# lijx10/SO-Net

Measured on AMD Instinct MI355X. Metric: point-clouds/sec forward, ModelNet40 5k-pt 8x8 SOM, higher is better.
Workload: dtype f32 (operands split into fp16 pieces, 3 fp16 MFMAs per product, f32 accumulate; parity 1e-5)

## Files before the change

include/sonet_hip.h:

```cpp
#ifndef SONET_HIP_H
#define SONET_HIP_H

#include <stddef.h>
#include <stdint.h>

#ifdef __cplusplus
extern "C" {
#endif

typedef void *sonet_stream_t;

enum {
    SONET_OK = 0,
    SONET_ERR_INVALID_ARG = 1,
    SONET_ERR_UNSUPPORTED = 2,
    SONET_ERR_LAUNCH = 3,
    SONET_ERR_NO_DEVICE = 4
};

int sonet_abi_version(void);
const char *sonet_build_arch(void);
const char *sonet_last_error(void);
int sonet_check_device(void);
int sonet_diag_mfma_f16_rate(int random_operands, int iters, double *tflops_out, double *ghz_out, sonet_stream_t stream);

int sonet_range_log_set(uint32_t *slot);

int sonet_index_max_f32(const float *data, const int32_t *index, int32_t *out_idx,
                        int B, int C, int Np, int K, sonet_stream_t stream);
int sonet_index_max_bf16(const uint16_t *data, const int32_t *index, int32_t *out_idx,
                         int B, int C, int Np, int K, sonet_stream_t stream);
int sonet_index_max_gather_f32(const float *data, const int32_t *index, const int32_t *row_max,
                               int32_t *out_idx, float *out_val,
                               int B, int C, int Np, int K, sonet_stream_t stream);
int sonet_index_max_gather_bf16(const uint16_t *data, const int32_t *index, const int32_t *row_max,
                                int32_t *out_idx, float *out_val, int B, int C, int Np, int K,
                                sonet_stream_t stream);
int sonet_index_max_gather_p16(const void *planes, const int32_t *index, const int32_t *row_max,
                               int32_t *out_idx, float *out_val, int B, int C, int Np, int K, sonet_stream_t stream);

int sonet_som_assign_f32(const float *x, const float *node, int B, int N, int M, int k,
                         int32_t *min_idx_i32, int64_t *min_idx_i64, int32_t *count, double *sum_ws,
                         sonet_stream_t stream);

int sonet_som_group_f32(const float *x, const float *sn, const int32_t *min_idx_i32,
                        const int32_t *count, const double *sum_ws, int B, int N, int M, int k,
                        float *som_node, int32_t *row_max, float *centers, float *x_decentered,
                        float *x_augmented, sonet_stream_t stream);

#define SONET_SOM_TRAIN_MAX_NODES 1024
#define SONET_SOM_TRAIN_MAX_POINTS (1 << 28)
int sonet_som_train_f32(const float *x, const float *node0, int node0_shared, const float *w, const float *lr,
                        int T, int B, int N, int M, float *node_out, sonet_stream_t stream);

int sonet_som_mask_i32(const int32_t *min_idx_i32, int32_t *mask, int B, int kN, int M,
                       sonet_stream_t stream);

int sonet_node_gather_f32(const float *feat, const int32_t *min_idx_i32, float *out,
                          int B, int C, int M, int kN, sonet_stream_t stream);

int sonet_knn_gather_f32(const float *x, const int64_t *knn_I, float *out,
                         int B, int C, int M, int K, sonet_stream_t stream);

int sonet_knn_self_f32(const float *node, int64_t *knn_I, int B, int M, int K, sonet_stream_t stream);

#define SONET_BATCH_SHAPENET 1
#define SONET_BATCH_TRAIN 2
#define SONET_BATCH_ROT_HORIZONTAL 4
#define SONET_BATCH_ROT_PERTURBATION 8
#define SONET_BATCH_TRANSLATION 16
#define SONET_BATCH_FLAG_MASK 31
#define SONET_BATCH_DRAW_SCALARS 8
#define SONET_BATCH_MAX_K 16
int sonet_assemble_batch_f32(const float *src, long long P, const int64_t *offsets, int S, const float *nodes_src,
                             const int64_t *idx, int B, int N, int M, int K, int flags, long long seed,
                             long long step, const int64_t *replay_idx, const double *replay_draws, double *draws_out,
                             float *pc, float *sn, float *node, int64_t *chosen, int64_t *knn_I, int32_t *bad,
                             sonet_stream_t stream);

int sonet_knn_group_f32(const float *coord, const float *feat, const int64_t *knn_I, int B, int C, int M, int K,
                        int center_avg, float *center, float *out, sonet_stream_t stream);
int sonet_knn_prepare_f32(const float *coord, const int64_t *knn_I, int B, int M, int K, int center_avg,
                          float *center, float *dec, int32_t *gidx, sonet_stream_t stream);
int sonet_pointmlp_h3_gather_f32(const float *x1, int C1, int L1, const int32_t *gidx, const float *x2, int C2, const void *Wp3,
                                 const float *scale, const float *shift, int relu, float *y,
                                 int B, int Cout, int L, sonet_stream_t stream);
int sonet_planes_max_f32(const float *x, float *out, long long rows, int K, int M, sonet_stream_t stream);

int sonet_lastdim_max_f32(const float *x, float *out, long long rows, int K, sonet_stream_t stream);

size_t sonet_pointmlp_pack_size(int Cin, int Cout);
int sonet_pointmlp_pack_f32(const float *W, float *Wp, int Cin, int Cout, sonet_stream_t stream);
int sonet_pointmlp_f32(const float *x1, int C1, const float *x2, int C2, const float *Wp,
                       const float *scale, const float *shift, int relu, float *y,
                       int B, int Cout, int L, sonet_stream_t stream);

int sonet_pointmlp_x3_bnb_f32(const float *gy, const float *raw, int C, const void *Wp3, const float *scale, const float *shift,
                              const float *a, const float *b, const float *c0, const float *sc, const float *sh, int relu,
                              float *g_raw_out, float *y, int B, int Cout, int L,
                              const float *praw, const float *psc, const float *psh, int prelu, void *pstats_ws, double *psums,
                              sonet_stream_t stream);

int sonet_pointmlp_x3_bnb_acc_f32(const float *gy, const float *raw, int C, const void *Wp3, const float *scale, const float *shift,
                                  const float *a, const float *b, const float *c0, const float *sc, const float *sh, int relu,
                                  float *g_raw_out, const float *yadd, float *y, int B, int Cout, int L, sonet_stream_t stream);

size_t sonet_pointmlp_x3_pack_size(int Cin, int Cout);
int sonet_pointmlp_x3_pack(const float *W, void *Wp3, int Cin, int Cout, sonet_stream_t stream);
int sonet_pointmlp_x3_f32(const float *x1, int C1, const float *x2, int C2, const void *Wp3,
                          const float *scale, const float *shift, int relu, float *y,
                          int B, int Cout, int L, sonet_stream_t stream);

int sonet_pointmlp_h3_pack(const float *W, void *Wp3, int Cin, int Cout, sonet_stream_t stream);
int sonet_pointmlp_h3_f32(const float *x1, int C1, const float *x2, int C2, const void *Wp3,
                          const float *scale, const float *shift, int relu, float *y,
                          int B, int Cout, int L, sonet_stream_t stream);

size_t sonet_p16_size(int B, int C, int L);
int sonet_p16_from_f32(const float *x, void *p16, int B, int C, int L, const float *scale, const float *shift, int relu,
                       sonet_stream_t stream);
int sonet_p16_to_f32(const void *p16, float *x, int B, int C, int L, sonet_stream_t stream);
size_t sonet_pointmlp_h3p_pack_size(int Cin, int Cout);
int sonet_pointmlp_h3p_pack(const float *W, void *Wp, int Cin, int Cout, sonet_stream_t stream);
size_t sonet_pointmlp_h3p_stats_ws_size(int B, int Cout, int L);
int sonet_pointmlp_h3p(const void *x1p, int C1, int L1, const int32_t *gidx, const void *x2p, int C2, const void *Wp,
                       const float *scale, const float *shift, int relu, float *y, void *yp, int B, int Cout, int L,
                       const float *zadd, const int32_t *zidx, int ZM, void *stats_ws, float *mean, float *var,
                       sonet_stream_t stream);

size_t sonet_knn_stage_columns(int B, int M, int K);
size_t sonet_node_stage_columns(int B, int M);
int sonet_knn_stage_prepare_f32(const float *coord, const int64_t *knn_I, int KI, int center_avg, int B, int M, int K,
                                float *center, void *center_p16, void *rec, sonet_stream_t stream);
int sonet_knn_stage_input_p16(const void *rec, const void *z_p16, const float *wl, const float *scale, const float *shift, int relu,
                              int B, int M, int K, int C, void *h1_p16, sonet_stream_t stream);
int sonet_pointmlp_h3p_gmax(const void *x1p, int C1, const void *x2p, int C2, const void *Wp, const float *scale, const float *shift,
                            int relu, int Cout, int L, int GK, int G, int ngout, int Lout, float *y, void *yp, sonet_stream_t stream);
int sonet_p16_flat_to_bcm_f32(const void *p16, float *x, int B, int C, int M, sonet_stream_t stream);

int sonet_lastdim_argmax_f32(const float *x, float *out, int32_t *idx, long long rows, int K, sonet_stream_t stream);
int sonet_lastdim_argmax_bf16(const uint16_t *x, uint16_t *out, int32_t *idx, long long rows, int K, sonet_stream_t stream);
int sonet_lastdim_max_bwd_f32(const float *g, const int32_t *idx, float *gx, long long rows, int K, sonet_stream_t stream);
int sonet_lastdim_max_bwd_bf16(const uint16_t *g, const int32_t *idx, uint16_t *gx, long long rows, int K, sonet_stream_t stream);
size_t sonet_knn_gather_bwd_ws_size(int B, int M, int K);
int sonet_knn_gather_bwd_f32(const float *g, const int64_t *knn_I, float *gx, void *ws, int B, int C, int M, int K, sonet_stream_t stream);
int sonet_knn_gather_bwd_bf16(const uint16_t *g, const int64_t *knn_I, float *gx, void *ws, int B, int C, int M, int K, sonet_stream_t stream);
size_t sonet_node_gather_bwd_ws_size(int B, int M, int L);
int sonet_node_gather_bwd_f32(const float *g, const int32_t *ids, float *gx, void *ws, int B, int C, int M, int L, sonet_stream_t stream);
int sonet_node_gather_bwd_bf16(const uint16_t *g, const int32_t *ids, float *gx, void *ws, int B, int C, int M, int L, sonet_stream_t stream);
size_t sonet_pointwise_bwd_apply_nodesum_ws_size(int B, int M, int L);
int sonet_pointwise_bwd_apply_nodesum_tile(void);
int sonet_pointwise_bwd_apply_nodesum_f32(const float *gy, const float *raw, const float *scale, const float *shift, int relu,
                                          const float *a, const float *b, const float *c0, const int32_t *ids, int M,
                                          float *g_raw, float *gz, void *ws, int B, int C, int L, sonet_stream_t stream);

size_t sonet_pointmlp_bf16_pack_size(int Cin, int Cout);
int sonet_pointmlp_bf16_pack(const float *W, void *Wp, int Cin, int Cout, sonet_stream_t stream);
int sonet_pointmlp_bf16(const uint16_t *x1, int C1, const uint16_t *x2, int C2, const void *Wp,
                        const float *scale, const float *shift, int relu, uint16_t *y,
                        int B, int Cout, int L, sonet_stream_t stream);
int sonet_pointmlp_bf16_gather(const uint16_t *x1, int C1, int L1, const int32_t *gidx, const uint16_t *x2, int C2, const void *Wp,
                               const float *scale, const float *shift, int relu, uint16_t *y,
                               int B, int Cout, int L, sonet_stream_t stream);
int sonet_pointmlp_bf16_acc(const uint16_t *x1, int C1, const uint16_t *x2, int C2, const void *Wp,
                            const float *scale, const float *shift, int relu, const uint16_t *yadd, uint16_t *y,
                            int B, int Cout, int L, sonet_stream_t stream);
int sonet_pointmlp_bf16_bnb(const uint16_t *gy, const uint16_t *raw, int C, const void *Wp, const float *scale, const float *shift,
                            const float *a, const float *b, const float *c0, const float *sc, const float *sh, int relu,
                            uint16_t *g_raw_out, const uint16_t *yadd, uint16_t *y, int B, int Cout, int L, sonet_stream_t stream);

size_t sonet_pointresnet_pack_size(void);
int sonet_pointresnet_pack(const float *W1, const float *W2, const float *W3, const float *W4, int Cin0,
                           void *wstream, sonet_stream_t stream);
int sonet_pointresnet_fused_f32(const float *x, int Cin0, const void *wstream, const float *affine,
                                float *y, int B, int L, sonet_stream_t stream);
int sonet_pointresnet_fused_p16_f32(const float *x, int Cin0, const void *wstream, const float *affine,
                                    float *y, void *yp, int B, int L, sonet_stream_t stream);

size_t sonet_pointresnet_bf16_pack_size(void);
int sonet_pointresnet_bf16_pack(const float *W1, const float *W2, const float *W3, const float *W4, int Cin0,
                                void *wstream, sonet_stream_t stream);
int sonet_pointresnet_bf16(const float *x, int Cin0, const void *wstream, const float *affine,
                           uint16_t *y, int B, int L, sonet_stream_t stream);

size_t sonet_pointresnet_bf16_pool_ws_size(int B, int L, int M);
int sonet_pointresnet_bf16_pool(const float *x_sorted, int Cin0, const void *wstream, const float *affine,
                                const int32_t *ids_sorted, const int32_t *pos0, const int32_t *node_off,
                                const int32_t *count, void *ws, float *out, int B, int L, int M, sonet_stream_t stream);

size_t sonet_pointresnet_pool_ws_size(int B, int L, int M);
int sonet_pointresnet_fused_pool_f32(const float *x_sorted, int Cin0, const void *wstream, const float *affine,
                                     const int32_t *ids_sorted, const int32_t *pos0, const int32_t *node_off,
                                     const int32_t *count, void *ws, float *out, int B, int L, int M, sonet_stream_t stream);
int sonet_pointresnet_fused_pool_p16_f32(const float *x_sorted, int Cin0, const void *wstream, const float *affine,
                                         const int32_t *ids_sorted, const int32_t *pos0, const int32_t *node_off,
                                         const int32_t *count, void *ws, float *out, void *out_p16, int B, int L, int M, sonet_stream_t stream);
size_t sonet_som_assign_sort_ws_size(int B, int N, int M, int k);
int sonet_som_assign_sort_f32(const float *x, const float *sn, const float *node, int B, int N, int M, int k,
                              int32_t *min_idx_i32, int64_t *min_idx_i64, int32_t *count, double *sum_ws,
                              float *som_node, int32_t *row_max, float *x_aug_sorted, int32_t *ids_sorted,
                              int32_t *pos0, int32_t *node_off, void *ws, sonet_stream_t stream);
int sonet_som_assign_sort_det_f32(const float *x, const float *sn, const float *node, int B, int N, int M, int k,
                              int32_t *min_idx_i32, int64_t *min_idx_i64, int32_t *count, double *sum_ws,
                              float *som_node, int32_t *row_max, float *x_aug_sorted, int32_t *ids_sorted,
                              int32_t *pos0, int32_t *node_off, void *ws, sonet_stream_t stream);
int sonet_som_assign_sort_knn_f32(const float *x, const float *sn, const float *node, int B, int N, int M, int k,
                                  int32_t *min_idx_i32, int64_t *min_idx_i64, int32_t *count, double *sum_ws,
                                  float *som_node, int32_t *row_max, float *x_aug_sorted, int32_t *ids_sorted,
                                  int32_t *pos0, int32_t *node_off, void *ws,
                                  const int64_t *knn_I, int KI, int K, int center_avg, float *center, void *center_p16, void *rec,
                                  sonet_stream_t stream);
int sonet_som_sort_group_f32(const float *x, const float *sn, const int32_t *min_idx_i32, const int32_t *count,
                             const double *sum_ws, int B, int N, int M, int k, float *som_node, int32_t *row_max,
                             float *x_aug_sorted, int32_t *ids_sorted, int32_t *pos0, int32_t *node_off,
                             int32_t *cursor_ws, sonet_stream_t stream);

int sonet_channel_stats_bf16(const uint16_t *y, int B, int C, int L, double *stat_ws, float *mean, float *var, sonet_stream_t stream);
int sonet_channel_affine_act_out_bf16(const uint16_t *x, const float *scale, const float *shift, int relu, uint16_t *y,
                                      int B, int C, int L, sonet_stream_t stream);
int sonet_pointwise_bwd_stats_bf16(const uint16_t *gy, const uint16_t *raw, const float *scale, const float *shift,
                                   int relu, int B, int C, int L, double *sums, sonet_stream_t stream);
int sonet_pointwise_bwd_apply_bf16(const uint16_t *gy, const uint16_t *raw, const float *scale, const float *shift, int relu,
                                   const float *a, const float *b, const float *c0, uint16_t *g_raw, int B, int C, int L,
                                   sonet_stream_t stream);

int sonet_pointwise_bwd_stats_f32(const float *gy, const float *raw, const float *scale, const float *shift,
                                  int relu, int B, int C, int L, double *sums, sonet_stream_t stream);
int sonet_pointwise_bwd_apply_f32(const float *gy, const float *raw, const float *scale, const float *shift, int relu,
                                  const float *a, const float *b, const float *c0, float *g_raw,
                                  int B, int C, int L, sonet_stream_t stream);
int sonet_node_add_affine_act_f32(float *t, const float *z, const int32_t *min_idx_i32, const float *scale,
                                  const float *shift, int relu, int B, int C, int L, int M, sonet_stream_t stream);

size_t sonet_pointmlp_stats_ws_size(int B, int Cout, int L);
int sonet_pointmlp_h3_stats_f32(const float *x1, int C1, const float *x2, int C2, const void *Wp3, const float *scale,
                                const float *shift, int relu, float *y, int B, int Cout, int L, void *stats_ws,
                                float *mean, float *var, sonet_stream_t stream);
int sonet_pointmlp_x3_stats_f32(const float *x1, int C1, const float *x2, int C2, const void *Wp3, const float *scale,
                                const float *shift, int relu, float *y, int B, int Cout, int L, void *stats_ws,
                                float *mean, float *var, sonet_stream_t stream);

int sonet_pointmlp_h3_nodeadd_f32(const float *x1, int C1, const float *x2, int C2, const void *Wp3, const float *scale,
                                  const float *shift, int relu, float *y, int B, int Cout, int L,
                                  const float *zadd, const int32_t *zidx, int ZM, sonet_stream_t stream);
int sonet_pointmlp_h3_nodeadd_stats_f32(const float *x1, int C1, const float *x2, int C2, const void *Wp3, const float *scale,
                                        const float *shift, int relu, float *y, int B, int Cout, int L,
                                        const float *zadd, const int32_t *zidx, int ZM, void *stats_ws,
                                        float *mean, float *var, sonet_stream_t stream);

size_t sonet_pointmlp_bf16_stats_ws_size(int B, int Cout, int L);
int sonet_pointmlp_bf16_stats(const uint16_t *x1, int C1, const uint16_t *x2, int C2, const void *Wp,
                              const float *scale, const float *shift, int relu, uint16_t *y,
                              int B, int Cout, int L, void *stats_ws, float *mean, float *var, sonet_stream_t stream);
int sonet_pointmlp_bf16_pool(const uint16_t *x1, int C1, const uint16_t *x2, int C2, const void *Wp,
                             const float *scale, const float *shift, int relu, const int32_t *ids, const int32_t *row_max,
                             int32_t *out_idx, float *out_val, int B, int Cout, int L, int M, sonet_stream_t stream);
int sonet_pointmlp_bf16_stats_xaff(const uint16_t *x1, int C1, const uint16_t *x2, int C2, const void *Wp,
                                   const float *scale, const float *shift, int relu, uint16_t *y,
                                   int B, int Cout, int L, void *stats_ws, float *mean, float *var,
                                   const float *xs1, const float *xh1, const float *xs2, const float *xh2, int xrelu,
                                   sonet_stream_t stream);
int sonet_pointmlp_bf16_pool_xaff(const uint16_t *x1, int C1, const uint16_t *x2, int C2, const void *Wp,
                                  const float *scale, const float *shift, int relu, const int32_t *ids, const int32_t *row_max,
                                  int32_t *out_idx, float *out_val, int B, int Cout, int L, int M,
                                  const float *xs1, const float *xh1, const float *xs2, const float *xh2, int xrelu,
                                  sonet_stream_t stream);

size_t sonet_pointmlp_h3_segpool_ws_size(int B, int Cout, int M);
int sonet_pointmlp_h3_segpool_f32(const float *x1, int C1, const float *x2, int C2, const void *Wp3, const float *scale,
                                  const float *shift, int relu, const int32_t *ids_sorted, const int32_t *pos0,
                                  const int32_t *row_max, int M, void *ws, int32_t *out_idx, float *out_val,
                                  int B, int Cout, int L, const float *xs1, const float *xh1, const float *xs2, const float *xh2,
                                  int xrelu, sonet_stream_t stream);
int sonet_pointmlp_h3_stats_xaff_f32(const float *x1, int C1, const float *x2, int C2, const void *Wp3, const float *scale,
                                     const float *shift, int relu, float *y, int B, int Cout, int L, void *stats_ws,
                                     float *mean, float *var, const float *xs1, const float *xh1, const float *xs2, const float *xh2,
                                     int xrelu, sonet_stream_t stream);

size_t sonet_wgrad_x3_ws_size(int B, int Cout, int Cin, int L);
int sonet_wgrad_x3_f32(const float *g, const float *x, float *dw, void *ws, int B, int Cout, int Cin, int L, sonet_stream_t stream);
int sonet_wgrad_x3_xaff_f32(const float *g, const float *x, float *dw, void *ws, int B, int Cout, int Cin, int L,
                            const float *xs, const float *xh, int xrelu, sonet_stream_t stream);
size_t sonet_wgrad_bf16_ws_size(int B, int Cout, int Cin, int L);
int sonet_wgrad_bf16(const uint16_t *g, const uint16_t *x, float *dw, void *ws, int B, int Cout, int Cin, int L, sonet_stream_t stream);
int sonet_wgrad_bf16_xaff(const uint16_t *g, const uint16_t *x, float *dw, void *ws, int B, int Cout, int Cin, int L,
                          const float *xs, const float *xh, int xrelu, sonet_stream_t stream);
int sonet_node_gather_lead_affine_act_f32(const float *z, const int32_t *gidx, const float *lead, const float *wl,
                                          const float *scale, const float *shift, int relu, float *out,
                                          int B, int C, int L, int M, int NL, sonet_stream_t stream);

// ... 122 lines not shown
```

so-net_amd/csrc/device.hpp:

```cpp
#pragma once
#include <hip/hip_runtime.h>
#include <stdint.h>
#include <type_traits>

typedef float f32x2_t __attribute__((ext_vector_type(2)));
typedef float f32x4_t __attribute__((ext_vector_type(4)));
typedef float f32x16 __attribute__((ext_vector_type(16)));
typedef _Float16 f16x2_t __attribute__((ext_vector_type(2)));
typedef _Float16 f16x8 __attribute__((ext_vector_type(8)));
typedef __bf16 bf16x8 __attribute__((ext_vector_type(8)));
typedef short i16x2 __attribute__((ext_vector_type(2)));
typedef int i32x4_t __attribute__((ext_vector_type(4)));
typedef unsigned u32x4_t __attribute__((ext_vector_type(4)));

template <int V> using int_c = std::integral_constant<int, V>;
template <bool B> using bool_c = std::integral_constant<bool, B>;

__device__ __forceinline__ unsigned cvt_pk_bf16(float lo, float hi) {
    unsigned r;
    asm("v_cvt_pk_bf16_f32 %0, %1, %2" : "=v"(r) : "v"(lo), "v"(hi));
    return r;
}
__device__ __forceinline__ unsigned cvt_pk_f16(float lo, float hi) {
    const f32x2_t v = {lo, hi};
    return __builtin_bit_cast(unsigned, __builtin_convertvector(v, f16x2_t));
}
__device__ __forceinline__ unsigned ord_f32(unsigned bits) {
    if (bits == 0x80000000u) bits = 0u;
    const unsigned o = bits ^ ((unsigned)((int)bits >> 31) | 0x80000000u);
    return (bits & 0x7FFFFFFFu) > 0x7F800000u ? 0u : o;
}

constexpr int RAW_BUFFER_WORD3 = 0x00020000;
template <typename T>
__device__ __forceinline__ __amdgpu_buffer_rsrc_t raw_buffer(const T *ptr, int bytes) {
    return __builtin_amdgcn_make_buffer_rsrc(const_cast<T *>(ptr), 0, bytes, RAW_BUFFER_WORD3);
}
__device__ __forceinline__ i32x4_t raw_buffer_sgpr(const void *base, unsigned bytes) {
    const unsigned long long a = reinterpret_cast<unsigned long long>(base);
    i32x4_t r;
    r[0] = __builtin_amdgcn_readfirstlane((int)(unsigned)a);
    r[1] = __builtin_amdgcn_readfirstlane((int)(unsigned)((a >> 32) & 0xFFFFu));
    r[2] = __builtin_amdgcn_readfirstlane((int)bytes);
    r[3] = RAW_BUFFER_WORD3;
    return r;
}

__device__ __forceinline__ float ld_f32(const float *p, long long i) { return p[i]; }
__device__ __forceinline__ float ld_f32(const uint16_t *p, long long i) { return __uint_as_float((unsigned)p[i] << 16); }
__device__ __forceinline__ void st_rne(float *p, long long i, float v) { p[i] = v; }
__device__ __forceinline__ void st_rne(uint16_t *p, long long i, float v) { p[i] = (uint16_t)(cvt_pk_bf16(v, v) & 0xFFFFu); }
__device__ __forceinline__ void st4_rne(float *o, const float (&v)[4]) { *reinterpret_cast<float4 *>(o) = make_float4(v[0], v[1], v[2], v[3]); }
__device__ __forceinline__ void st4_rne(uint16_t *o, const float (&v)[4]) {
    *reinterpret_cast<uint2 *>(o) = make_uint2(cvt_pk_bf16(v[0], v[1]), cvt_pk_bf16(v[2], v[3]));
}

__device__ __forceinline__ unsigned bf16_pair_affine_act(unsigned pk, f32x2_t sc, f32x2_t sh, unsigned floor2) {
    const f32x2_t x = {__uint_as_float(pk << 16), __uint_as_float(pk & 0xFFFF0000u)};
    f32x2_t v;
    asm("v_pk_fma_f32 %0, %1, %2, %3" : "=v"(v) : "v"(x), "v"(sc), "v"(sh));
    unsigned r = cvt_pk_bf16(v[0], v[1]);
    asm("v_pk_max_i16 %0, %1, %2" : "=v"(r) : "v"(r), "v"(floor2));
    return r;
}

__device__ __forceinline__ float row32_sum(float v) {
    v += __builtin_bit_cast(float, __builtin_amdgcn_update_dpp(0, __builtin_bit_cast(int, v), 0xB1, 0xF, 0xF, true));
    v += __builtin_bit_cast(float, __builtin_amdgcn_update_dpp(0, __builtin_bit_cast(int, v), 0x4E, 0xF, 0xF, true));
    v += __builtin_bit_cast(float, __builtin_amdgcn_update_dpp(0, __builtin_bit_cast(int, v), 0x141, 0xF, 0xF, true));
    v += __builtin_bit_cast(float, __builtin_amdgcn_update_dpp(0, __builtin_bit_cast(int, v), 0x140, 0xF, 0xF, true));
    v += __builtin_bit_cast(float, __builtin_amdgcn_ds_swizzle(__builtin_bit_cast(int, v), 0x401F));
    return v;
}

__device__ __forceinline__ int xcd_remap(int bid, int nwg) {
    const int q = nwg / sonet::NUM_XCD, r = nwg % sonet::NUM_XCD;
    const int xcd = bid % sonet::NUM_XCD, local = bid / sonet::NUM_XCD;
    const int base = xcd < r ? xcd * (q + 1) : r * (q + 1) + (xcd - r) * q;
    return base + local;
}

struct RangeAcc { int mp; unsigned mn; };
__device__ __forceinline__ void range_track(RangeAcc &r, float x0, float x1) {
    const int a = __float_as_int(x0), b = __float_as_int(x1);
    r.mp = max(max(r.mp, a), b);
    r.mn = max(max(r.mn, (unsigned)a), (unsigned)b);
}
__device__ __forceinline__ unsigned range_amax_bits(const RangeAcc &r) {
    const unsigned neg = (r.mn & 0x80000000u) ? (r.mn & 0x7FFFFFFFu) : 0u;
    const unsigned pos = (unsigned)r.mp;
    return pos > neg ? pos : neg;
}
__device__ __forceinline__ unsigned wave_umax(unsigned v) {
#pragma unroll
    for (int o = 32; o > 0; o >>= 1) { const unsigned t = (unsigned)__shfl_xor((int)v, o, 64); v = t > v ? t : v; }
    return v;
}
__device__ __forceinline__ void range_publish(unsigned *word, unsigned wave_max_bits, int lane) {
    if (lane == 0 && wave_max_bits > __atomic_load_n(word, __ATOMIC_RELAXED)) atomicMax(word, wave_max_bits);
}

__device__ __forceinline__ void p16_split2(float X0, float X1, unsigned &h, unsigned &m) {
    h = cvt_pk_f16(X0, X1);
    const f16x2_t hv = __builtin_bit_cast(f16x2_t, h);
    m = cvt_pk_f16(X0 - (float)hv[0], X1 - (float)hv[1]);
}
__device__ __forceinline__ void p16_split_pair(float x0, float x1, unsigned &h, unsigned &m) {
    p16_split2(32.f * __builtin_amdgcn_fmed3f(x0, -2047.f, 2047.f), 32.f * __builtin_amdgcn_fmed3f(x1, -2047.f, 2047.f), h, m);
}
__device__ __forceinline__ float clamp_keep_nan(float w, float lim) { return w < -lim ? -lim : (w > lim ? lim : w); }
__device__ __forceinline__ int p16_channel(int h, int e) { return 4 * h + (e & 3) + 8 * (e >> 2); }

__device__ __forceinline__ void split3_pair(float x0, float x1, unsigned &h, unsigned &m, unsigned &l) {
    h = cvt_pk_bf16(x0, x1);
    const float r0 = x0 - __uint_as_float(h << 16), r1 = x1 - __uint_as_float(h & 0xFFFF0000u);
    m = cvt_pk_bf16(r0, r1);
    const float q0 = r0 - __uint_as_float(m << 16), q1 = r1 - __uint_as_float(m & 0xFFFF0000u);
    l = cvt_pk_bf16(q0, q1);
}

__device__ __forceinline__ void split3_fix_w(float w, unsigned &h, unsigned &m, unsigned &l) {
    if ((h & 0x7FFFu) != 0x7F80u) return;
    if (__builtin_isinf(w)) { l = h; h = 0u; m = 0u; return; }
    h -= 1u;
    const float r = w - __uint_as_float(h << 16);
    m = cvt_pk_bf16(r, 0.f) & 0xFFFFu;
    l = cvt_pk_bf16(r - __uint_as_float(m << 16), 0.f) & 0xFFFFu;
}
__device__ __forceinline__ void split3_pair_w(float w0, float w1, unsigned &h, unsigned &m, unsigned &l) {
    split3_pair(w0, w1, h, m, l);
    unsigned h0 = h & 0xFFFFu, m0 = m & 0xFFFFu, l0 = l & 0xFFFFu, h1 = h >> 16, m1 = m >> 16, l1 = l >> 16;
    split3_fix_w(w0, h0, m0, l0);
    split3_fix_w(w1, h1, m1, l1);
    h = h0 | (h1 << 16); m = m0 | (m1 << 16); l = l0 | (l1 << 16);
}

__device__ __forceinline__ float cluster_mean(float sum, float count) { return __fdiv_rn(sum, __fadd_rn(count, 1e-5f)); }
```

so-net_amd/csrc/node_stage.hip:

```cpp
#include "common.hpp"

namespace {

constexpr int KS_CPW = 4;

__global__ __launch_bounds__(256) void knn_stage_prepare_kernel(const float *__restrict__ coord, const int64_t *__restrict__ I, int KI, int avg,
                                                                 int B, int M, int K, int G, long long Lp, long long Lm,
                                                                 float *__restrict__ center, uint4 *__restrict__ center_p16, int4 *__restrict__ rec,
                                                                 unsigned *__restrict__ rlog)
{
    const long long l = (long long)blockIdx.x * 256 + threadIdx.x;
    if (l >= Lp) return;
    const int col = (int)(l & 127);
    const long long BM = (long long)B * M;
    const int g = col / K, k = col - g * K;
    const long long n = (l >> 7) * G + g;
    if (!(g < G && n < BM)) {
        rec[l] = make_int4(-2, 0, 0, 0);
        return;
    }
    const int b = (int)(n / M), m = (int)(n - (long long)b * M);
    const int64_t *Ib = I + ((long long)b * M + m) * KI;
    const float *cb = coord + (long long)b * 3 * M;
    const long long id = Ib[k];
    const bool ok = (unsigned long long)id < (unsigned long long)M;
    float d[3], ctr[3];
#pragma unroll
    for (int c = 0; c < 3; ++c) {
        const float *src = cb + c * M;
        if (avg) {
            float sum = 0.f;
            for (int kk = 0; kk < K; ++kk) {
                const long long ik = Ib[kk];
                sum += ((unsigned long long)ik < (unsigned long long)M) ? src[ik] : 0.f;
            }
            ctr[c] = sum / (float)K;
        } else {
            ctr[c] = src[m];
        }
        d[c] = (ok ? src[id] : 0.f) - ctr[c];
    }
    rec[l] = make_int4(ok ? (int)((long long)b * M + id) : -1, __float_as_int(d[0]), __float_as_int(d[1]), __float_as_int(d[2]));
    if (k == 0) {
#pragma unroll
        for (int c = 0; c < 3; ++c) center[((long long)b * 3 + c) * M + m] = ctr[c];
        unsigned h0, m0, h1v, m1;
        p16_split_pair(ctr[0], ctr[1], h0, m0);
        p16_split_pair(ctr[2], 0.f, h1v, m1);
        center_p16[(0 * 2 + 0) * Lm + n] = make_uint4(h0, h1v, 0u, 0u);
        center_p16[(0 * 2 + 1) * Lm + n] = make_uint4(0u, 0u, 0u, 0u);
        center_p16[(1 * 2 + 0) * Lm + n] = make_uint4(m0, m1, 0u, 0u);
        center_p16[(1 * 2 + 1) * Lm + n] = make_uint4(0u, 0u, 0u, 0u);
        if (rlog != nullptr) {
            RangeAcc xr = {0, 0u};
            range_track(xr, ctr[0], ctr[1]);
            range_track(xr, ctr[2], 0.f);
            const unsigned bits = range_amax_bits(xr);
            if (bits > __atomic_load_n(rlog + 2, __ATOMIC_RELAXED)) atomicMax(rlog + 2, bits);
        }
    }
}


constexpr int KS_MAXG = 8;

__global__ __launch_bounds__(256) void knn_stage_input_kernel(const int4 *__restrict__ rec, const uint4 *__restrict__ zp, const float *__restrict__ wl,
                                                               const float *__restrict__ scale, const float *__restrict__ shift, int relu,
                                                               int C, long long Lp, long long Lm, uint4 *__restrict__ h1, unsigned *__restrict__ rlog, int abl)
{
    __shared__ unsigned wmax[4];
    __shared__ __attribute__((aligned(16))) float coef[5][KS_MAXG * KS_CPW * 16];
    const int col = threadIdx.x & 127;
    const int hh = __builtin_amdgcn_readfirstlane((int)(threadIdx.x >> 7));
    const long long lcol = (long long)blockIdx.x * 128 + col;
    const int4 r = rec[lcol];
    const int KC = (C + 15) >> 4;
    const int ngrp = (KC + KS_CPW - 1) / KS_CPW, gstride = (int)gridDim.y;
    for (int t = threadIdx.x; t < KS_MAXG * KS_CPW * 16; t += 256) {
        const int j = t >> 6, i = (t >> 4) & 3, h = (t >> 3) & 1, e = t & 7;
        const int grp = (int)blockIdx.y + j * gstride;
        const int c = (grp * KS_CPW + i) * 16 + p16_channel(h, e);
        const bool in = grp < ngrp && c < C;
        coef[0][t] = in ? 32.f * wl[c * 3 + 0] : 0.f;
        coef[1][t] = in ? 32.f * wl[c * 3 + 1] : 0.f;
        coef[2][t] = in ? 32.f * wl[c * 3 + 2] : 0.f;
        coef[3][t] = in ? scale[c] : 0.f;
        coef[4][t] = in ? 32.f * shift[c] : 0.f;
    }
    const bool valid = r.x != -2, ok = r.x >= 0;
    const f32x2_t d0 = {__int_as_float(r.y), __int_as_float(r.y)}, d1 = {__int_as_float(r.z), __int_as_float(r.z)},
                d2 = {__int_as_float(r.w), __int_as_float(r.w)};
    RangeAcc xr = {0, 0u};
    const float lo = relu ? 0.f : -65504.f;
    const uint4 *zbase = zp + (long long)hh * Lm + (ok ? r.x : 0);
    uint4 *hbase = h1 + (long long)hh * Lp + lcol;

    auto load = [&](uint4 (&zh)[KS_CPW], uint4 (&zm)[KS_CPW], int grp) {
        const uint4 *zq = zbase + (long long)(grp * KS_CPW) * 4 * Lm;
#pragma unroll
        for (int i = 0; i < KS_CPW; ++i) {
            zh[i] = make_uint4(0u, 0u, 0u, 0u);
            zm[i] = zh[i];
#ifdef SONET_VARIANTS
            if (abl & 2) { zh[i] = make_uint4(r.y, r.z, r.w, r.x); zm[i] = zh[i]; } else
#endif
            if (ok && grp * KS_CPW + i < KC) {
                zh[i] = zq[0];
                zm[i] = zq[2 * Lm];
            }
            zq += 4 * Lm;
        }
    };
    auto process = [&](const uint4 (&zhq)[KS_CPW], const uint4 (&zmq)[KS_CPW], int grp, int j) {
        uint4 *hq = hbase + (long long)(grp * KS_CPW) * 4 * Lp;
#pragma unroll
        for (int i = 0; i < KS_CPW; ++i) {
            if (grp * KS_CPW + i >= KC) break;
            const unsigned zh[4] = {zhq[i].x, zhq[i].y, zhq[i].z, zhq[i].w}, zm[4] = {zmq[i].x, zmq[i].y, zmq[i].z, zmq[i].w};
            unsigned hv[4], mv[4];
#pragma unroll
            for (int q = 0; q < 4; ++q) {
                const int slot = (j * KS_CPW + i) * 16 + hh * 8 + 2 * q;
                const f32x2_t w0 = *reinterpret_cast<const f32x2_t *>(&coef[0][slot]), w1 = *reinterpret_cast<const f32x2_t *>(&coef[1][slot]),
                            w2 = *reinterpret_cast<const f32x2_t *>(&coef[2][slot]), sc = *reinterpret_cast<const f32x2_t *>(&coef[3][slot]),
                            sh = *reinterpret_cast<const f32x2_t *>(&coef[4][slot]);
                const f16x2_t zh2 = __builtin_bit_cast(f16x2_t, zh[q]), zm2 = __builtin_bit_cast(f16x2_t, zm[q]);
                f32x2_t a = __builtin_convertvector(zh2, f32x2_t) + __builtin_convertvector(zm2, f32x2_t);
                a = __builtin_elementwise_fma(w0, d0, a);
                a = __builtin_elementwise_fma(w1, d1, a);
                a = __builtin_elementwise_fma(w2, d2, a);
                a = __builtin_elementwise_fma(a, sc, sh);
                if (!valid) a = f32x2_t{0.f, 0.f};
                range_track(xr, a[0], a[1]);
                p16_split2(__builtin_amdgcn_fmed3f(a[0], lo, 65504.f), __builtin_amdgcn_fmed3f(a[1], lo, 65504.f), hv[q], mv[q]);
            }
#ifdef SONET_VARIANTS
            if ((abl & 1) && hv[0] != 0x12345u) { hq += 4 * Lp; continue; }
#endif
            hq[0] = make_uint4(hv[0], hv[1], hv[2], hv[3]);
            hq[2 * Lp] = make_uint4(mv[0], mv[1], mv[2], mv[3]);
            hq += 4 * Lp;
        }
    };

    uint4 zhA[KS_CPW], zmA[KS_CPW], zhB[KS_CPW], zmB[KS_CPW];
    int grp = (int)blockIdx.y, j = 0;
    load(zhA, zmA, grp);
    __syncthreads();
    for (; grp < ngrp; grp += 2 * gstride, j += 2) {
        const bool more = grp + gstride < ngrp;
        if (more) load(zhB, zmB, grp + gstride);
        process(zhA, zmA, grp, j);
        if (more) {
            if (grp + 2 * gstride < ngrp) load(zhA, zmA, grp + 2 * gstride);
            process(zhB, zmB, grp + gstride, j + 1);
        }
    }
    if (rlog != nullptr) {
        unsigned bits;
        if (relu) {
            const unsigned pos = xr.mp > 0 ? (unsigned)xr.mp : 0u, nan_neg = xr.mn > 0xFF800000u ? (xr.mn & 0x7FFFFFFFu) : 0u;
            bits = pos > nan_neg ? pos : nan_neg;
        } else {
            bits = range_amax_bits(xr);
        }
        unsigned wm = wave_umax(bits);
        wm = wm > (5u << 23) ? wm - (5u << 23) : 0u;
        if ((threadIdx.x & 63) == 0) wmax[threadIdx.x >> 6] = wm;
        __syncthreads();
        if (threadIdx.x == 0) {
            const unsigned a = wmax[0] > wmax[1] ? wmax[0] : wmax[1], c2 = wmax[2] > wmax[3] ? wmax[2] : wmax[3];
            const unsigned mx = a > c2 ? a : c2;
            if (mx > __atomic_load_n(rlog + 2, __ATOMIC_RELAXED)) atomicMax(rlog + 2, mx);
        }
    }
}

__global__ __launch_bounds__(256) void p16_flat_to_bcm_kernel(const uint4 *__restrict__ p, float *__restrict__ x, int C, int M, long long BM, long long Lm, int KC)
{
    const long long l = (long long)blockIdx.x * 256 + threadIdx.x;
    const int kc = blockIdx.y >> 1, hh = blockIdx.y & 1;
    if (l >= BM) return;
    const uint4 hv = p[((long long)(kc * 2 + 0) * 2 + hh) * Lm + l], mv = p[((long long)(kc * 2 + 1) * 2 + hh) * Lm + l];
    const f16x8 h8 = __builtin_bit_cast(f16x8, hv), m8 = __builtin_bit_cast(f16x8, mv);
    const long long b = l / M;
    const int m = (int)(l - b * M);
#pragma unroll
    for (int e = 0; e < 8; ++e) {
        const int c = kc * 16 + p16_channel(hh, e);
        if (c < C) x[(b * C + c) * M + m] = ((float)h8[e] + (float)m8[e]) * 0.03125f;
    }
}

}

extern "C" size_t sonet_knn_stage_columns(int B, int M, int K)
{
    if (B <= 0 || M <= 0 || K <= 0 || K > 128) return 0;
    return (size_t)(sonet::ceil_div64((long long)B * M, knn_stage_groups(K)) * 128);
}

extern "C" size_t sonet_node_stage_columns(int B, int M)
{
    if (B <= 0 || M <= 0) return 0;
    return (size_t)(sonet::ceil_div64((long long)B * M, 128) * 128);
}

extern "C" int sonet_knn_stage_prepare_f32(const float *coord, const int64_t *knn_I, int KI, int center_avg, int B, int M, int K,
                                           float *center, void *center_p16, void *rec, sonet_stream_t stream)
{
    const char *what = "sonet_knn_stage_prepare_f32";
    SONET_REQUIRE(coord && knn_I && center && center_p16 && rec, "%s: NULL pointer", what);
    SONET_REQUIRE(B > 0 && M > 0 && K >= 1 && K <= 128 && KI >= K, "%s: bad size B=%d M=%d K=%d (of %d)", what, B, M, K, KI);
    const long long Lp = (long long)sonet_knn_stage_columns(B, M, K), Lm = (long long)sonet_node_stage_columns(B, M);
    if (Lp / 256 + 1 > 0x7FFFFFFFll) return sonet::fail(SONET_ERR_UNSUPPORTED, "%s: too many columns", what);
    hipLaunchKernelGGL(knn_stage_prepare_kernel, dim3((unsigned)sonet::ceil_div64(Lp, 256)), dim3(256), 0, sonet::as_stream(stream),
                       coord, knn_I, KI, center_avg, B, M, K, knn_stage_groups(K), Lp, Lm, center, reinterpret_cast<uint4 *>(center_p16),
                       reinterpret_cast<int4 *>(rec), sonet::range_log());
    return sonet::launched(what);
}

extern "C" int sonet_knn_stage_input_p16(const void *rec, const void *z_p16, const float *wl, const float *scale, const float *shift, int relu,
                                         int B, int M, int K, int C, void *h1_p16, sonet_stream_t stream)
{
    const char *what = "sonet_knn_stage_input_p16";
    SONET_REQUIRE(rec && z_p16 && wl && scale && shift && h1_p16, "%s: NULL pointer", what);
    SONET_REQUIRE(B > 0 && M > 0 && C > 0 && K >= 1 && K <= 128, "%s: bad size B=%d M=%d C=%d K=%d", what, B, M, C, K);
    const long long Lp = (long long)sonet_knn_stage_columns(B, M, K), Lm = (long long)sonet_node_stage_columns(B, M);
    const long long nblk = Lp / 128;
    const int KC = sonet::ceil_div(C, 16);
    if (nblk > 0x7FFFFFFFll || (double)KC * 64.0 * (double)Lp >= 2.0e9) return sonet::fail(SONET_ERR_UNSUPPORTED, "%s: too many columns", what);
    const int ngrp = sonet::ceil_div(KC, KS_CPW);
    int gy = sonet::ceil_div(ngrp, KS_MAXG);
    while (gy < ngrp && nblk * gy < 512) ++gy;
#ifdef SONET_VARIANTS
    if (const char *e = sonet::knob("SONET_KSI_GY")) { const int v = atoi(e); if (v >= sonet::ceil_div(ngrp, KS_MAXG) && v <= ngrp) gy = v; }
#endif
    hipLaunchKernelGGL(knn_stage_input_kernel, dim3((unsigned)nblk, (unsigned)gy), dim3(256), 0, sonet::as_stream(stream),
                       reinterpret_cast<const int4 *>(rec), reinterpret_cast<const uint4 *>(z_p16), wl, scale, shift, relu, C, Lp, Lm,
                       reinterpret_cast<uint4 *>(h1_p16), sonet::range_log(), sonet::knob("SONET_KSI_ABL") ? atoi(sonet::knob("SONET_KSI_ABL")) : 0);
    return sonet::launched(what);
}

extern "C" int sonet_p16_flat_to_bcm_f32(const void *p16, float *x, int B, int C, int M, sonet_stream_t stream)
{
    const char *what = "sonet_p16_flat_to_bcm_f32";
    SONET_REQUIRE(p16 && x, "%s: NULL pointer", what);
    SONET_REQUIRE(B > 0 && C > 0 && M > 0, "%s: non-positive size", what);
    const int KC = sonet::ceil_div(C, 16);
    const long long BM = (long long)B * M;
    if (KC * 2 > 65535) return sonet::fail(SONET_ERR_UNSUPPORTED, "%s: C too large for one launch", what);
    hipLaunchKernelGGL(p16_flat_to_bcm_kernel, dim3((unsigned)sonet::ceil_div64(BM, 256), (unsigned)(KC * 2)), dim3(256), 0, sonet::as_stream(stream),
                       reinterpret_cast<const uint4 *>(p16), x, C, M, BM, (long long)sonet_node_stage_columns(B, M), KC);
    return sonet::launched(what);
}
```

so-net_amd/csrc/pointmlp_h3p.hip:

```cpp
#include "common.hpp"

namespace {

constexpr int P_THREADS = 256;
constexpr int P_KPAD = 8;
constexpr unsigned OOB = 0x7FFFFF00u;

template <bool RELU>
__device__ __forceinline__ void split_act(float x0, float x1, unsigned &h, unsigned &m) {
    constexpr float lo = RELU ? 0.f : -2047.f;
    p16_split2(32.f * __builtin_amdgcn_fmed3f(x0, lo, 2047.f), 32.f * __builtin_amdgcn_fmed3f(x1, lo, 2047.f), h, m);
}

__global__ __launch_bounds__(256) void h3p_pack_kernel(const float *__restrict__ W, uint4 *__restrict__ Wp, int Cin, int Cout, int KCP,
                                                        long long total, unsigned *__restrict__ trailer)
{
    const long long t = (long long)blockIdx.x * 256 + threadIdx.x;
    if (t >= total) return;
    RangeAcc wr = {0, 0u};
    const int lane = (int)(t & 63);
    const long long r = t >> 6;
    const int kc = (int)(r % KCP), ct = (int)(r / KCP);
    const int o = ct * 32 + (lane & 31), hh = lane >> 5;
    unsigned h[4], m[4];
#pragma unroll
    for (int p = 0; p < 4; ++p) {
        const int c0 = kc * 16 + p16_channel(hh, 2 * p), c1 = c0 + 1;
        float w0 = (o < Cout && c0 < Cin) ? W[(long long)o * Cin + c0] : 0.f;
        float w1 = (o < Cout && c1 < Cin) ? W[(long long)o * Cin + c1] : 0.f;
        range_track(wr, w0, w1);
        w0 = 32.f * clamp_keep_nan(w0, 2047.f);
        w1 = 32.f * clamp_keep_nan(w1, 2047.f);
        p16_split2(w0, w1, h[p], m[p]);
    }
    uint4 *dst = Wp + (r * 2) * 64 + lane;
    dst[0] = make_uint4(h[0], h[1], h[2], h[3]);
    dst[64] = make_uint4(m[0], m[1], m[2], m[3]);
    range_publish(trailer, wave_umax(range_amax_bits(wr)), lane);
}

template <bool AFFINE>
__global__ __launch_bounds__(256) void p16_from_f32_kernel(const float *__restrict__ x, uint4 *__restrict__ p, int C, int L, int KC,
                                                            const float *__restrict__ scale, const float *__restrict__ shift, int relu,
                                                            unsigned *__restrict__ rlog)
{
    __shared__ unsigned wmax[4];
    const int kc = blockIdx.y >> 1, hh = blockIdx.y & 1, b = blockIdx.z;
    RangeAcc xr = {0, 0u};
    const float *xb0 = x + (size_t)b * C * L;
    uint4 *pb = p + (size_t)b * KC * 4 * L;
    float sc[8], sf[8];
    if constexpr (AFFINE) {
#pragma unroll
        for (int e = 0; e < 8; ++e) {
            const int c = kc * 16 + p16_channel(hh, e);
            sc[e] = c < C ? scale[c] : 0.f;
            sf[e] = c < C ? shift[c] : 0.f;
        }
    }
#pragma unroll
    for (int it = 0; it < 4; ++it) {
        const int l = blockIdx.x * 1024 + it * 256 + threadIdx.x;
        if (l >= L) break;
        const float *xb = xb0 + l;
        float v[8];
#pragma unroll
        for (int e = 0; e < 8; ++e) {
            const int c = kc * 16 + p16_channel(hh, e);
            float t = c < C ? xb[(size_t)c * L] : 0.f;
            if constexpr (AFFINE) {
                t = __fmaf_rn(t, sc[e], sf[e]);
                if (relu) t = t < 0.f ? 0.f : t;
            }
            v[e] = t;
        }
        unsigned h[4], m[4];
#pragma unroll
        for (int q = 0; q < 4; ++q) {
            range_track(xr, v[2 * q], v[2 * q + 1]);
            split_act<false>(v[2 * q], v[2 * q + 1], h[q], m[q]);
        }
        pb[((size_t)(kc * 2 + 0) * 2 + hh) * L + l] = make_uint4(h[0], h[1], h[2], h[3]);
        pb[((size_t)(kc * 2 + 1) * 2 + hh) * L + l] = make_uint4(m[0], m[1], m[2], m[3]);
    }
    if (rlog != nullptr) {
        const unsigned wm = wave_umax(range_amax_bits(xr));
        if ((threadIdx.x & 63) == 0) wmax[threadIdx.x >> 6] = wm;
        __syncthreads();
        if (threadIdx.x == 0) {
            const unsigned a = wmax[0] > wmax[1] ? wmax[0] : wmax[1], c2 = wmax[2] > wmax[3] ? wmax[2] : wmax[3];
            const unsigned mx = a > c2 ? a : c2;
            if (mx > __atomic_load_n(rlog + 2, __ATOMIC_RELAXED)) atomicMax(rlog + 2, mx);
        }
    }
}

__global__ __launch_bounds__(256) void p16_to_f32_kernel(const uint4 *__restrict__ p, float *__restrict__ x, int C, int L, int KC)
{
    const int l = blockIdx.x * 256 + threadIdx.x;
    const int kc = blockIdx.y >> 1, hh = blockIdx.y & 1, b = blockIdx.z;
    if (l >= L) return;
    const uint4 *pb = p + (size_t)b * KC * 4 * L;
    const uint4 hv = pb[((size_t)(kc * 2 + 0) * 2 + hh) * L + l], mv = pb[((size_t)(kc * 2 + 1) * 2 + hh) * L + l];
    const f16x8 h8 = __builtin_bit_cast(f16x8, hv), m8 = __builtin_bit_cast(f16x8, mv);
    float *xb = x + (size_t)b * C * L + l;
#pragma unroll
    for (int e = 0; e < 8; ++e) {
        const int c = kc * 16 + p16_channel(hh, e);
        if (c < C) xb[(size_t)c * L] = ((float)h8[e] + (float)m8[e]) * 0.03125f;
    }
}

struct H3pArgs {
    const void *x1, *x2;
    const void *Wp;
    const float *scale, *shift;
    float *y;
    void *yp;
    const int32_t *gidx;
    const float *zadd;
    const int32_t *zidx;
    unsigned *rlog;
    double *stats_partial;
    int abl;
    unsigned long long *prof;
    long long ngroups;
    int KC1, KC2, L1, L, Cout, CT, KC, KCr, KCP, ct_per_y, nslab, ncol, gpc, relu, ZM;
    int GK, G, ngout, Lout;
};

__device__ __forceinline__ u32x4_t bload16(i32x4_t rsrc, unsigned voff, unsigned soff) {
    u32x4_t r;
    asm volatile("buffer_load_dwordx4 %0, %1, %2, %3 offen" : "=v"(r) : "v"(voff), "s"(rsrc), "s"(soff) : "memory");
    return r;
}
__device__ __forceinline__ void bstore16(__amdgpu_buffer_rsrc_t rsrc, unsigned voff, unsigned soff, u32x4_t v) {
    __builtin_amdgcn_raw_buffer_store_b128(v, rsrc, voff, soff, 0);
}
__device__ __forceinline__ void bstore4(__amdgpu_buffer_rsrc_t rsrc, unsigned voff, unsigned soff, float v) {
    __builtin_amdgcn_raw_buffer_store_b32(__builtin_bit_cast(unsigned, v), rsrc, voff, soff, 0);
}
template <int N>
__device__ __forceinline__ void wait_barrier(u32x4_t &a, u32x4_t &b) {
    asm volatile("s_waitcnt vmcnt(%2)\n\ts_barrier" : "+v"(a), "+v"(b) : "n"(N) : "memory");
}
template <int N>
__device__ __forceinline__ void wait_barrier(u32x4_t &a, u32x4_t &b, u32x4_t &c, u32x4_t &d) {
    asm volatile("s_waitcnt vmcnt(%4)\n\ts_barrier" : "+v"(a), "+v"(b), "+v"(c), "+v"(d) : "n"(N) : "memory");
}

template <int NC>
__device__ __forceinline__ void sched_pair() {
    __builtin_amdgcn_sched_group_barrier(0x100, 1, 0);
    __builtin_amdgcn_sched_group_barrier(0x008, NC == 2 ? 3 : 1, 0);
    __builtin_amdgcn_sched_group_barrier(0x100, 1, 0);
    __builtin_amdgcn_sched_group_barrier(0x008, NC == 2 ? 3 : 2, 0);
    __builtin_amdgcn_sched_group_barrier(0x100, 1, 0);
    __builtin_amdgcn_sched_group_barrier(0x008, NC == 2 ? 3 : 1, 0);
    __builtin_amdgcn_sched_group_barrier(0x100, 1, 0);
    __builtin_amdgcn_sched_group_barrier(0x008, NC == 2 ? 3 : 2, 0);
}

constexpr int GM_STRIDE = 136;
__device__ __forceinline__ float nan_max(float m, float v) { return (v > m || v != v) ? v : m; }
__device__ __forceinline__ void lds_barrier() { asm volatile("s_waitcnt lgkmcnt(0)\n\ts_barrier" ::: "memory"); }

template <int MT, int NC, int OCC, int EPI, int OUT>
__global__ __launch_bounds__(P_THREADS, OCC) void pointmlp_h3p_kernel(const H3pArgs a)
{
    static_assert(OUT >= 1 && OUT <= 3 && (EPI != 2 || (OUT & 1)), "output mode");
    static_assert(EPI < 4 || (NC == 1 && ((EPI == 4 && OUT == 2) || (EPI == 5 && OUT == 1))), "group-max epilogues: 32-column waves, P16 (4) or f32 (5) out");
    static_assert(MT % 2 == 0 && (NC == 1 || NC == 2), "tile shape");
    constexpr int PB = (OCC >= 2 && NC == 2 && (EPI == 1 || EPI == 3)) ? 2 : 3, NB = 4, D = 3, NSLOT = D + 2;
    static_assert(D >= PB && PB >= 2, "the wait count below assumes the W request of a chunk is older than its X request");
    constexpr int NSL = MT * 2;
    constexpr int ND = NSL / 4;
    constexpr int NBL = NC * 2;
    constexpr int NP = MT / 2;
    constexpr int KWAIT = (PB - 1) * (NBL + ND);
    static_assert(KWAIT < 64, "vmcnt is a 6-bit counter");
    struct Lds {
        u32x4_t wsm[NSLOT][NSL][64];
        float aff[EPI == 1 ? 1024 : 2048];
        float2 red[EPI == 2 ? 4 : 1][EPI == 2 ? MT * 32 : 1];
        float zl[EPI == 1 ? MT * 32 : 1][EPI == 1 ? 64 : 1];
        float gm[EPI >= 4 ? 32 : 1][EPI >= 4 ? GM_STRIDE : 1];
    };
    __shared__ __attribute__((aligned(16))) Lds lds;

    const int wg_xcd = blockIdx.x & 7, wg_local = blockIdx.x >> 3;
    const int wg_col = (wg_local / a.nslab) * 8 + wg_xcd, wg_slab = wg_local - (wg_local / a.nslab) * a.nslab;
    if (wg_col >= a.ncol) return;

    const int lane = threadIdx.x & 63;
    const int wave = __builtin_amdgcn_readfirstlane(threadIdx.x >> 6);
    const int j = lane & 31, h = lane >> 5;
    long long q = (long long)wg_col * 4 + wave;
    const bool wave_valid = q < a.ngroups;
    q = wave_valid ? q : 0;
    const int b = __builtin_amdgcn_readfirstlane((int)(q / a.gpc));
    const int l0 = __builtin_amdgcn_readfirstlane((int)(q - (long long)b * a.gpc) * (32 * NC));
    const int L = a.L, L1 = a.L1;

    bool pv[NC];
    unsigned vo1[NC], vo2[NC], voy[NC], voyp[NC];
    int lcl[NC];
#pragma unroll
    for (int c = 0; c < NC; ++c) {
        const int l = l0 + 32 * c + j;
        pv[c] = wave_valid && l < L;
        lcl[c] = l < L ? l : l0;
        vo2[c] = (unsigned)(h * L + lcl[c]) * 16u;
        vo1[c] = (unsigned)(h * L1 + lcl[c]) * 16u;
        if (a.gidx) {
            const int src = a.gidx[(size_t)b * L + lcl[c]];
            vo1[c] = (unsigned)src < (unsigned)L1 ? (unsigned)(h * L1 + src) * 16u : OOB;
        }
        voy[c] = pv[c] ? (unsigned)(4 * h * L + l) * 4u : OOB;
        voyp[c] = pv[c] ? (unsigned)(h * L + l) * 16u : OOB;
#ifdef SONET_VARIANTS
        if (a.abl & 1) { voy[c] = OOB; voyp[c] = OOB; pv[c] = false; }
#endif
    }
    const i32x4_t r1 = raw_buffer_sgpr(static_cast<const char *>(a.x1) + (size_t)b * a.KC1 * 64 * L1, (unsigned)a.KC1 * 64u * (unsigned)L1);
    const i32x4_t r2 = raw_buffer_sgpr(a.x2 ? static_cast<const char *>(a.x2) + (size_t)b * a.KC2 * 64 * L : static_cast<const char *>(a.x1),
                                 a.x2 ? (unsigned)a.KC2 * 64u * (unsigned)L : 0u);
    const __amdgpu_buffer_rsrc_t ry = __builtin_amdgcn_make_buffer_rsrc(
        a.y ? reinterpret_cast<char *>(a.y) + (size_t)b * a.Cout * L * 4 : nullptr, 0, a.y ? (int)((unsigned)a.Cout * (unsigned)L * 4u) : 0, RAW_BUFFER_WORD3);
    const __amdgpu_buffer_rsrc_t ryp = __builtin_amdgcn_make_buffer_rsrc(
        a.yp ? static_cast<char *>(a.yp) + (size_t)b * (a.Cout / 16) * 64 * L : nullptr, 0, a.yp ? (int)((unsigned)(a.Cout / 16) * 64u * (unsigned)L) : 0, RAW_BUFFER_WORD3);

    const int ct_begin = wg_slab * a.ct_per_y;
    const int ct_end = min(a.CT, ct_begin + a.ct_per_y);
    const int npass = (ct_end - ct_begin) / MT;
    const int KCr = a.KCr, KC1 = a.KC1;
#ifdef SONET_VARIANTS
    unsigned long long pt0 = __builtin_readcyclecounter(), pt_loop = 0, pt_epi = 0, pt_pro = 0;
#endif
    const unsigned wsm_lds = (unsigned)reinterpret_cast<size_t>(&lds.wsm[0][0][0]);
    const unsigned vow = (unsigned)lane * 16u;
    const char *wp = static_cast<const char *>(a.Wp);

    auto load_b = [&](u32x4_t (&bb)[NBL], int kc) {
#ifdef SONET_VARIANTS
        if (a.abl & 2) kc = 0;
#endif
        const bool second = kc >= KC1;
        const int kk = second ? kc - KC1 : kc;
        const unsigned rowb = (unsigned)(second ? L : L1) * 32u;
        const i32x4_t rs = second ? r2 : r1;
#pragma unroll
        for (int c = 0; c < NC; ++c) {
            const unsigned vo = second ? vo2[c] : vo1[c];
            bb[2 * c + 0] = bload16(rs, vo, (unsigned)(kk * 2 + 0) * rowb);
            bb[2 * c + 1] = bload16(rs, vo, (unsigned)(kk * 2 + 1) * rowb);
        }
    };
    auto dma = [&](int pass, int kc, int slot) {
#ifdef SONET_VARIANTS
        if (a.abl & 4) { kc = 0; pass = 0; }
#endif
        const int ps = pass < npass ? pass : npass - 1;
        const char *g0 = wp + ((size_t)(ct_begin + ps * MT) * a.KCP + kc) * 2048u;
        const unsigned d0 = wsm_lds + (unsigned)slot * (unsigned)(NSL * 1024);
#pragma unroll
        for (int t = 0; t < ND; ++t) {
            const int sl = wave + 4 * t;
            const char *g = g0 + (size_t)(sl >> 1) * ((size_t)a.KCP * 2048u) + (size_t)(sl & 1) * 1024u;
            const unsigned d = d0 + (unsigned)sl * 1024u;
            unsigned keep;
            asm volatile("s_mov_b32 %0, m0\n\ts_mov_b32 m0, %3\n\ts_nop 4\n\tglobal_load_lds_dwordx4 %1, %2\n\ts_mov_b32 m0, %0"
                         : "=&s"(keep) : "v"(vow), "s"(g), "s"(d) : "memory");
        }
    };
    auto read_a = [&](u32x4_t (&A)[4], int slot, int p) {
#pragma unroll
        for (int u = 0; u < 4; ++u) A[u] = lds.wsm[slot][4 * p + u][lane];
    };

    f32x16 acc[MT][NC];

    auto mfma_pair = [&](const u32x4_t (&A)[4], const u32x4_t (&bb)[NBL], int p) {
        f16x8 Bh[NC], Bm[NC];
#pragma unroll
        for (int c = 0; c < NC; ++c) {
            Bh[c] = __builtin_bit_cast(f16x8, bb[2 * c + 0]);
            Bm[c] = __builtin_bit_cast(f16x8, bb[2 * c + 1]);
        }
#pragma unroll
        for (int term = 0; term < 3; ++term)
#pragma unroll
            for (int tt = 0; tt < 2; ++tt)
#pragma unroll
                for (int c = 0; c < NC; ++c)
                {
                    const f16x8 wf = __builtin_bit_cast(f16x8, A[2 * tt + (term == 0 ? 1 : 0)]), xf = term == 1 ? Bm[c] : Bh[c];
                    acc[2 * p + tt][c] = __builtin_amdgcn_mfma_f32_32x32x16_f16(wf, xf, acc[2 * p + tt][c], 0, 0, 0);
                }
    };

    RangeAcc yr = {0, 0u};
    const float relu_thr = a.relu ? 0.f : -__builtin_inff();
    const float split_lo = a.relu ? 0.f : -2047.f;
    int zm[NC];
    bool zok[NC];
    unsigned zvo[NC], zla[NC];
    const i32x4_t rz = raw_buffer_sgpr(a.zadd ? a.zadd + (size_t)b * a.Cout * a.ZM : nullptr, a.zadd ? (unsigned)a.Cout * (unsigned)a.ZM * 4u : 0u);
    if constexpr (EPI == 1 || EPI == 3) {
#pragma unroll
        for (int c = 0; c < NC; ++c) {
            zm[c] = a.zidx[(size_t)b * L + lcl[c]];
            zok[c] = (unsigned)zm[c] < (unsigned)a.ZM;
            zm[c] = zok[c] ? zm[c] : 0;
            zvo[c] = zok[c] ? (unsigned)(zm[c] + 4 * h * a.ZM) * 4u : OOB;
            zla[c] = (unsigned)reinterpret_cast<size_t>(&lds.zl[4 * h][zm[c]]);
            asm volatile("" : "+v"(zla[c]));
        }
    }
    auto epilogue = [&](int ct0) {
        if constexpr (EPI >= 4) {
#pragma unroll
            for (int mt = 0; mt < MT; ++mt) {
                if ((ct0 + mt) * 32 >= a.Cout) continue;
                float asc16[16], ash16[16];
                {
                    const float4 *t4 = reinterpret_cast<const float4 *>(lds.aff + (ct0 - ct_begin + mt) * 64 + h * 32);
#pragma unroll
                    for (int u = 0; u < 4; ++u) {
                        const float4 s4 = t4[u], h4 = t4[4 + u];
                        asc16[4 * u] = s4.x; asc16[4 * u + 1] = s4.y; asc16[4 * u + 2] = s4.z; asc16[4 * u + 3] = s4.w;
                        ash16[4 * u] = h4.x; ash16[4 * u + 1] = h4.y; ash16[4 * u + 2] = h4.z; ash16[4 * u + 3] = h4.w;
                    }
                }
                __builtin_amdgcn_sched_barrier(0);
#pragma unroll
                for (int r = 0; r < 16; ++r) {
                    const float v = __fmaf_rn(acc[mt][0][r], asc16[r], ash16[r]);
                    lds.gm[(r & 3) + 8 * (r >> 2) + 4 * h][32 * wave + j] = v < relu_thr ? 0.f : v;
                }
                lds_barrier();
                const int t = (int)threadIdx.x;
                if constexpr (EPI == 4) {
                    const int p = t & 3, u = t >> 2;
                    const int g = u % a.G, qh = u / a.G;
                    if (qh < 4) {
                        const int qq = qh >> 1, h2 = qh & 1;
                        const float *r0 = &lds.gm[16 * qq + 4 * h2 + 2 * (p & 1) + 8 * (p >> 1)][g * a.GK];
                        float m0 = r0[0], m1 = r0[GM_STRIDE];
                        for (int k = 1; k < a.GK; ++k) {
                            m0 = nan_max(m0, r0[k]);
                            m1 = nan_max(m1, r0[GM_STRIDE + k]);
                        }
                        const long long n_out = (long long)wg_col * a.G + g;
                        if (n_out < a.ngout) {
                            range_track(yr, m0, m1);
                            unsigned hv, mv;
                            p16_split2(__builtin_amdgcn_fmed3f(m0, split_lo * 32.f, 65504.f), __builtin_amdgcn_fmed3f(m1, split_lo * 32.f, 65504.f), hv, mv);
                            unsigned *dst = reinterpret_cast<unsigned *>(static_cast<char *>(a.yp)
                                + ((((size_t)((ct0 + mt) * 2 + qq) * 2) * 2 + h2) * (size_t)a.Lout + (size_t)n_out) * 16) + p;
                            dst[0] = hv;
                            dst[(size_t)a.Lout * 8] = mv;
                        }
                    }
                } else {
                    const int seg = t & 3, row = (t >> 2) & 31, g = t >> 7;
                    const int cols = a.GK >> 2;
                    const float *r0 = &lds.gm[row][(g < a.G ? g : 0) * a.GK + seg * cols];
                    float m = r0[0];
                    for (int k = 1; k < cols; ++k) m = nan_max(m, r0[k]);
                    m = nan_max(m, __builtin_bit_cast(float, __builtin_amdgcn_update_dpp(0, __builtin_bit_cast(int, m), 0xB1, 0xF, 0xF, true)));
                    m = nan_max(m, __builtin_bit_cast(float, __builtin_amdgcn_update_dpp(0, __builtin_bit_cast(int, m), 0x4E, 0xF, 0xF, true)));
                    const long long n_out = (long long)wg_col * a.G + g;
                    if (seg == 0 && g < a.G && n_out < a.ngout) a.y[(size_t)n_out * a.Cout + (size_t)(ct0 + mt) * 32 + row] = m;
                }
                lds_barrier();
            }
            return;
        }
#pragma unroll
        for (int mt = 0; mt < MT; ++mt) {
            if ((ct0 + mt) * 32 >= a.Cout) continue;
            float asc16[16], ash16[16];
            {
                const float4 *t4 = reinterpret_cast<const float4 *>(lds.aff + (ct0 - ct_begin + mt) * 64 + h * 32);
#pragma unroll
                for (int u = 0; u < 4; ++u) {
                    const float4 s4 = t4[u], h4 = t4[4 + u];
                    asc16[4 * u] = s4.x; asc16[4 * u + 1] = s4.y; asc16[4 * u + 2] = s4.z; asc16[4 * u + 3] = s4.w;
                    ash16[4 * u] = h4.x; ash16[4 * u + 1] = h4.y; ash16[4 * u + 2] = h4.z; ash16[4 * u + 3] = h4.w;
                }
            }
            __builtin_amdgcn_sched_barrier(0);
            float st1[EPI == 2 ? 16 : 1], st2[EPI == 2 ? 16 : 1];
#pragma unroll
            for (int c = 0; c < NC; ++c) {
#pragma unroll
                for (int qq = 0; qq < 2; ++qq) {
                    unsigned hh[4], mm[4];
#pragma unroll
                    for (int hf = 0; hf < 2; ++hf) {
                        const int r0 = 8 * qq + 4 * hf;
                        const int row0 = mt * 32 + 16 * qq + 8 * hf;
                        float av[4], v[4], zg[4];
#pragma unroll
                        for (int e = 0; e < 4; ++e) {
                            if constexpr (OCC == 1) asm volatile("v_accvgpr_read_b32 %0, %1" : "=v"(av[e]) : "a"(acc[mt][c][r0 + e]));
                            else av[e] = acc[mt][c][r0 + e];
                        }
                        if constexpr (EPI == 3) {
#pragma unroll
                            for (int e = 0; e < 4; ++e) {
                                const unsigned so = (unsigned)((ct0 + mt) * 32 + 16 * qq + 8 * hf + e) * (unsigned)a.ZM * 4u;
                                asm volatile("buffer_load_dword %0, %1, %2, %3 offen" : "=v"(zg[e]) : "v"(zvo[c]), "s"(rz), "s"(so) : "memory");
                            }
                            asm volatile("s_waitcnt vmcnt(0)" : "+v"(zg[0]), "+v"(zg[1]), "+v"(zg[2]), "+v"(zg[3]) :: "memory");
                        }
                        if constexpr (EPI == 1) {
#pragma unroll
                            for (int e = 0; e < 4; ++e)
                                asm volatile("v_add_u32 %0, %2, %1\n\tds_read_b32 %0, %0" : "=&v"(zg[e]) : "v"(zla[c]), "s"((row0 + e) * 256) : "memory");
                            asm volatile("s_waitcnt lgkmcnt(0)" : "+v"(zg[0]), "+v"(zg[1]), "+v"(zg[2]), "+v"(zg[3]) :: "memory");
                        }
#pragma unroll
                        for (int e = 0; e < 4; ++e) {
                            const float sc = asc16[r0 + e], sf = ash16[r0 + e];
                            if constexpr (EPI == 1 || EPI == 3) {
                                const float zv = EPI == 1 ? (zok[c] ? zg[e] : 0.f) : zg[e];
                                v[e] = __fmaf_rn(av[e], sc, __fmaf_rn(zv, sc * 1024.f, sf));
                            } else {
                                v[e] = __fmaf_rn(av[e], sc, sf);
                            }
                        }
                        if constexpr ((OUT & 1) != 0) {
#pragma unroll
                            for (int e = 0; e < 4; ++e) {
                                const int orow = 16 * qq + 8 * hf + e;
                                const float o = v[e] < relu_thr ? 0.f : v[e];
                                bstore4(ry, voy[c], (unsigned)((ct0 + mt) * 32 + orow) * (unsigned)L * 4u, o);
                                if constexpr (EPI == 2) {
                                    const float vv = pv[c] ? o : 0.f;
                                    st1[r0 + e] = c == 0 ? vv : st1[r0 + e] + vv;
                                    st2[r0 + e] = c == 0 ? vv * vv : st2[r0 + e] + vv * vv;
                                }
                            }
                        }
                        if constexpr ((OUT & 2) != 0) {
#pragma unroll
                            for (int p = 0; p < 2; ++p) {
                                const float x0 = v[2 * p], x1 = v[2 * p + 1];
                                range_track(yr, x0, x1);
                                if constexpr (OUT == 2)
                                    p16_split2(__builtin_amdgcn_fmed3f(x0, split_lo * 32.f, 65504.f), __builtin_amdgcn_fmed3f(x1, split_lo * 32.f, 65504.f),
                                           hh[2 * hf + p], mm[2 * hf + p]);
                                else
                                    p16_split2(32.f * __builtin_amdgcn_fmed3f(x0, split_lo, 2047.f), 32.f * __builtin_amdgcn_fmed3f(x1, split_lo, 2047.f),
                                           hh[2 * hf + p], mm[2 * hf + p]);
                            }
                        }
                        if constexpr (EPI == 1 || EPI == 3 || OUT == 3) __builtin_amdgcn_sched_barrier(0);
                    }
                    if constexpr ((OUT & 2) == 0) __builtin_amdgcn_sched_barrier(0);
                    if constexpr ((OUT & 2) != 0) {
                        const unsigned so = (unsigned)(((ct0 + mt) * 2 + qq) * 2) * (unsigned)L * 32u;
                        const u32x4_t hv = {hh[0], hh[1], hh[2], hh[3]}, mv = {mm[0], mm[1], mm[2], mm[3]};
                        bstore16(ryp, voyp[c], so, hv);
                        bstore16(ryp, voyp[c], so + (unsigned)L * 32u, mv);
                        __builtin_amdgcn_sched_barrier(0);
                    }
                }
            }
            if constexpr (EPI == 2) {
#pragma unroll
                for (int r = 0; r < 16; ++r) {
                    const float s1 = row32_sum(st1[r]), s2 = row32_sum(st2[r]);
                    if (j == 0) lds.red[wave][mt * 32 + (r & 3) + 8 * (r >> 2) + 4 * h] = make_float2(s1, s2);
                }
                __builtin_amdgcn_sched_barrier(0);
            }
        }
        if constexpr (EPI == 2) {
            __syncthreads();
            for (int t = threadIdx.x; t < MT * 32 && ct0 * 32 + t < a.Cout; t += P_THREADS) {
                const double s = ((double)lds.red[0][t].x + (double)lds.red[1][t].x) + ((double)lds.red[2][t].x + (double)lds.red[3][t].x);
                const double qq = ((double)lds.red[0][t].y + (double)lds.red[1][t].y) + ((double)lds.red[2][t].y + (double)lds.red[3][t].y);
                double *dst = a.stats_partial + ((size_t)wg_col * a.Cout + (size_t)ct0 * 32 + t) * 2;
                dst[0] = s;
                dst[1] = qq;
            }
            __syncthreads();
        }
        if constexpr (EPI == 1) __syncthreads();
    };
    auto z_dma = [&](int ct0) {
        if constexpr (EPI == 1) {
            {
                const char *g0 = reinterpret_cast<const char *>(a.zadd + ((size_t)b * a.Cout + (size_t)ct0 * 32) * 64);
                const unsigned d0 = (unsigned)reinterpret_cast<size_t>(&lds.zl[0][0]);
#pragma unroll
                for (int t = 0; t < MT * 2; ++t) {
                    const int piece = wave + 4 * t;
                    const char *g = g0 + (size_t)piece * 1024u;
                    const unsigned d = d0 + (unsigned)piece * 1024u;
                    unsigned keep;
                    asm volatile("s_mov_b32 %0, m0\n\ts_mov_b32 m0, %3\n\ts_nop 4\n\tglobal_load_lds_dwordx4 %1, %2\n\ts_mov_b32 m0, %0"
                                 : "=&s"(keep) : "v"(vow), "s"(g), "s"(d) : "memory");
                }
            }
        }
    };

    u32x4_t bq[NB][NBL];
    u32x4_t Aq[2][4];
#pragma unroll
    for (int i = 0; i <= D - PB; ++i) dma(0, i, i);
// ... 287 lines not shown
```

so-net_amd/models/networks.py:

```python
import math

import weakref

import torch
import torch.nn as nn

from sonet_hip import ops as _ops
from util import som
from .layers import EquivariantLayer, KNNModule, MyLinear, PointNet, PointResNet, _NodewiseLayerFn, _PlainAttrs


def _head_inference(fn):
    import functools

    @functools.wraps(fn)
    def wrapper(self, *args, **kwargs):
        ts = [a for a in args if isinstance(a, torch.Tensor) and a.is_floating_point()]
        dev = ts[0].device if ts else torch.device("cpu")
        if torch.is_grad_enabled() and not self.training and getattr(self, "inference", True):
            if ts and not any(t.requires_grad for t in ts) and any(getattr(t, "_sonet_inference", False) for t in ts):
                with torch.no_grad():
                    return _ops.mark_inference(_ops.run_guarded(lambda: fn(self, *args, **kwargs), dev, True))
        return _ops.run_guarded(lambda: fn(self, *args, **kwargs), dev, not (torch.is_grad_enabled() or self.training))
    return wrapper
# ... 49 lines not shown
            self.knnlayer = KNNModule(3 + 384, (512, 512), activation=act, normalization=norm, **kw)
            self.final_pointnet = PointNet(3 + 512, (768, self.feature_num), activation=act, normalization=norm, **kw)
        else:
            self.final_pointnet = PointResNet(3 + 384, (512, 512, 768, self.feature_num),
                                              activation=act, normalization=norm, **kw)
        rows = int(math.sqrt(opt.node_num))
        self.som_builder = som.BatchSOM(rows, rows, 3, opt.gpu_id, opt.batch_size)
        self.zero_pad = torch.nn.ZeroPad2d(padding=1)
        self._lazy = None
        self._first_pn_out = None

    @property
    def mask(self):
        st = self._lazy
        if st is None:
            raise AttributeError("Encoder.mask: call forward first")
        if st.get("mask") is None:
            st["mask"] = _ops.som_mask(st["a"].min_idx_i32, st["a"].M)
        return st["mask"]

    @property
    def min_idx(self):
        st = self._lazy
        if st.get("min_idx") is None:
            st["min_idx"] = st["a"].min_idx_i32.long()
        return st["min_idx"]

    def _per_point(self, name):
        st = self._lazy
        if st is None:
            raise AttributeError("Encoder.%s: call forward first" % name)
        if st.get(name) is None:
            g = _ops.som_group(st["x"], None, st["a"], want_centers=True, want_decentered=True)
            st["centers"], st["x_decentered"] = g["centers"], g["x_decentered"]
        return _ops.mark_inference(st[name]) if getattr(self, "_infer_tag", False) else st[name]

    @property
    def first_pn_out(self):
        if self._first_pn_out is None and self._lazy is not None and self._lazy.get("first_p16") is not None:
            self._first_pn_out = self._lazy["first_p16"].float()
        if self._first_pn_out is None and self._lazy is not None and self._lazy.get("not_materialised"):
            raise RuntimeError("Encoder.first_pn_out was not materialised by this training forward (only its per-node maximum is consumed: the "
                               "pool ran in the last layer's epilogue); set encoder.want_first_pn_out = True before the forward to keep it")
        if self._first_pn_out is None and self._lazy is not None:
            st = self._lazy
            g = _ops.som_group(st["x"], st["sn"], st["a"], want_augmented=st["sn"] is not None, want_decentered=st["sn"] is None)
            with torch.no_grad():
                self._first_pn_out = self.first_pointnet(g["x_augmented"] if st["sn"] is not None else g["x_decentered"], None)
        if getattr(self, "_infer_tag", False):
            _ops.mark_inference(self._first_pn_out)
        return self._first_pn_out

    @first_pn_out.setter
    def first_pn_out(self, v):
        self._first_pn_out = v

    def _stage_map(self, name):
        v = self.__dict__.get("_" + name)
        st = self.__dict__.get("_stage")
        if v is None and st is not None:
            with torch.no_grad():
                if name == "knn_feature_1":
                    v = _ops.p16_flat_to_bcm(st["knn_p16"], st["B"], st["M"])
                else:
                    lyr = self.final_pointnet.layers[1]
                    sc, sh = lyr._eval_affine()
                    y = _ops.pointmlp_h3p(st["h3_p16"], lyr._packed_p16(), sc, sh, lyr.activation == 'relu', lyr.conv.out_channels, out="f32")
                    v = y[0, :, :st["B"] * st["M"]].reshape(-1, st["B"], st["M"]).permute(1, 0, 2).contiguous()
            if getattr(self, "_infer_tag", False):
                _ops.mark_inference(v)
            self.__dict__["_" + name] = v
        return v

    @property
    def knn_feature_1(self):
        return self._stage_map("knn_feature_1")

    @knn_feature_1.setter
    def knn_feature_1(self, v):
        self.__dict__["_knn_feature_1"] = v

    @property
    def final_pn_out(self):
        return self._stage_map("final_pn_out")

    @final_pn_out.setter
    def final_pn_out(self, v):
        self.__dict__["_final_pn_out"] = v

    @property
    def centers(self):
        return self._per_point("centers")

    @property
    def x_decentered(self):
        return self._per_point("x_decentered")

    def forward(self, x, sn, node=None, node_knn_I=None, is_train=False, epoch=None):
        if node is None or node_knn_I is None:
            node, node_knn_I = self._raw_cloud_nodes(x, node, node_knn_I)
        infer = (not is_train) and (not self.training) and getattr(self, "inference", True) and not x.requires_grad
        if infer and torch.is_grad_enabled():
            with torch.no_grad():
                out = self._forward_guarded(x, sn, node, node_knn_I, is_train, epoch)
        else:
            out = self._forward_guarded(x, sn, node, node_knn_I, is_train, epoch)
        self._infer_tag = (not torch.is_grad_enabled()) or infer
        if self._infer_tag:
            for t in (out, self.first_pn_out_masked_max, self.__dict__.get("_final_pn_out"), self.som_node, self.__dict__.get("_knn_feature_1")):
                _ops.mark_inference(t)
        return out

    def _raw_cloud_nodes(self, x, node, node_knn_I):
        with torch.no_grad():
            if node is None:
                self.som_builder.optimize(x.detach())
                node = self.som_builder.node
            if node_knn_I is None:
                node_knn_I = _ops.knn_self(node.detach().float().contiguous(), int(self.opt.som_k))
        return node, node_knn_I

    def _wants_dense(self):
        v = self.__dict__.get('want_first_pn_out')
        return bool(v) if v is not None else len(_DENSE_HEADS) > 0

    def _node_stage_ok(self, B, M, node_knn_I):
        opt = self.opt
        if not (_ops.NODE_STAGE_P16 and _ops.GATHER_NODE_STAGE and _ops.P16_CHAINS and _ops.POINTMLP_PRECISION == "h3" and opt.som_k >= 2) \
                or torch.is_grad_enabled():
            return False
        if getattr(self, 'want_first_pn_out', False):
            return False
        if M not in (64, 128) or node_knn_I is None or node_knn_I.dim() != 3 or node_knn_I.dtype != torch.int64 \
                or node_knn_I.shape[2] < opt.som_k or opt.som_k > 128 or opt.som_k_type not in ('avg', 'center'):
            return False
        if not isinstance(self.final_pointnet, PointNet) or len(self.knnlayer.layers) != 2 or len(self.final_pointnet.layers) != 2:
            return False
        k1, k2 = self.knnlayer.layers
        f1, f2 = self.final_pointnet.layers
        if k1.conv.in_channels != 3 + 384 or k2.conv.in_channels != k1.conv.out_channels or k1.conv.out_channels % 16 != 0 \
                or f1.conv.in_channels != 3 + k2.conv.out_channels or k2.conv.out_channels % 16 != 0 or f2.conv.in_channels != f1.conv.out_channels:
            return False
        return all(l._p16_ok() for l in (k1, k2, f1, f2))

    def _node_stage(self, xp, prep, B, M):
        K, G = prep["K"], prep["G"]
        k1, k2 = self.knnlayer.layers
        f1, f2 = self.final_pointnet.layers
        dev = xp.device
        C1 = k1.conv.out_channels
        z = _ops.pointmlp_h3p(xp, k1._packed_p16(lambda: k1._weight2d().detach()[:, 3:], "feat"), _ops.const_vec(C1, 1.0, dev),
                              _ops.const_vec(C1, 0.0, dev), False, C1, out="p16", tag="flat")
        s1, t1 = k1._eval_affine()
        h1 = _ops.knn_stage_input(prep, z, k1._lead_cols(3), s1, t1, k1.activation == 'relu')
        center, cp = prep["center"], prep["center_p16"]
        s2, t2 = k2._eval_affine()
        knn = _ops.pointmlp_h3p_gmax(h1, k2._packed_p16(), s2, t2, k2.activation == 'relu', k2.conv.out_channels, K, G, B * M, out="p16", Lout=xp.L)
        s3, t3 = f1._eval_affine()
        h3 = _ops.pointmlp_h3p(knn, f1._packed_p16(lambda: torch.cat((f1._weight2d().detach()[:, 3:], f1._weight2d().detach()[:, :3]), dim=1), "rot3"),
                               s3, t3, f1.activation == 'relu', f1.conv.out_channels, x2=cp, out="p16", tag="flat")
        s4, t4 = f2._eval_affine()
        feature = _ops.pointmlp_h3p_gmax(h3, f2._packed_p16(), s4, t4, f2.activation == 'relu', f2.conv.out_channels, M, 128 // M, B, out="f32")
        self.knn_center_1 = center
        self.__dict__["_stage"] = dict(knn_p16=knn, h3_p16=h3, B=B, M=M)
        self.__dict__["_knn_feature_1"] = None
        self.__dict__["_final_pn_out"] = None
        return feature

    def _forward_guarded(self, x, sn, node, node_knn_I, is_train, epoch):
        can_rerun = not (torch.is_grad_enabled() or self.training)
        return _ops.run_guarded(lambda: self._forward(x, sn, node, node_knn_I, is_train, epoch), x.device, can_rerun)

    def _forward(self, x, sn, node, node_knn_I, is_train=False, epoch=None):
        opt = self.opt
        M = node.size()[2]
        xd = x.detach().float().contiguous()
        sb = self.som_builder
        sb.node = node.detach().float().contiguous()
        use_sn = bool(opt.surface_normal)
        snd = sn.detach().float().contiguous() if use_sn else None
        fused_pool = (use_sn and _ops.FUSE_POOL and not getattr(self, 'want_first_pn_out', False)
                      and not torch.is_grad_enabled() and self.first_pointnet._fusable_eval(xd)
                      and int(opt.k) * xd.shape[2] * 384 * 4 < 4e9)
        stage = fused_pool and _ops.POINTMLP_PRECISION == "h3" and self._node_stage_ok(xd.shape[0], M, node_knn_I)
        knn = (node_knn_I.contiguous(), int(opt.som_k), opt.som_k_type == 'avg') if stage else None
        fast = sb.assign_sort(xd, snd, opt.k, knn=knn) if fused_pool else None
        if fast is not None:
            a, g = fast
        elif fused_pool:
            a = sb.assign(xd, opt.k)
            g = _ops.som_sort_group(xd, snd, a)
        else:
            a, g = None, None
        if fused_pool:
            sb.node = g["som_node"]
            self.som_node = sb.node
            self._lazy = dict(a=a, x=xd, sn=snd, mask=None, min_idx=None, centers=None, x_decentered=None)
            self._first_pn_out = None
            wstream, affine = self.first_pointnet._fused_state()
            self.__dict__["_stage"] = None
            if stage:
                prep = g.get("knn_prep")
                if prep is None:
                    prep = _ops.knn_stage_prepare(self.som_node, knn[0], knn[1], knn[2])
                self.first_pn_out_masked_max, xp = _ops.pointresnet_fused_pool(g, wstream, affine, M, want_p16=True)
                self.feature = self._node_stage(xp, prep, xd.shape[0], M)
                return self.feature
            pool = _ops.pointresnet_bf16_pool if _ops.POINTMLP_PRECISION == "bf16" else _ops.pointresnet_fused_pool
            self.first_pn_out_masked_max = pool(g, wstream, affine, M)
        else:
            self.__dict__["_stage"] = None
            train_pooled = torch.is_grad_enabled() and isinstance(self.first_pointnet, PointResNet) and getattr(self, "pooled_backward", True)
            per_point = self._wants_dense() if torch.is_grad_enabled() else bool(getattr(self, 'want_first_pn_out', False))
            sorted_pool = (train_pooled and use_sn and not per_point and a is None and self.first_pointnet.pooled_sorted_ok(xd, M)
                           and int(opt.k) * xd.shape[2] * 384 * 4 < 4e9)
            if sorted_pool:
                fast = sb.assign_sort(xd, snd, opt.k, deterministic=True) if _ops.TRAIN_ASSIGN_SORT else None
                if fast is not None:
                    a, g = fast
                else:
                    a = sb.assign(xd, opt.k)
                    g = _ops.som_sort_group(xd, snd, a)
                self._lazy = dict(a=a, x=xd, sn=snd, mask=None, min_idx=None, centers=None, x_decentered=None)
                pn_in = g["x_aug_sorted"]
            else:
                if a is None:
                    a = sb.assign(xd, opt.k)
                g = _ops.som_group(xd, snd, a, want_centers=per_point, want_decentered=(not use_sn) or per_point, want_augmented=use_sn)
                self._lazy = dict(a=a, x=xd, sn=snd, mask=None, min_idx=None,
                                  centers=g["centers"], x_decentered=g["x_decentered"])
                pn_in = g["x_augmented"] if use_sn else g["x_decentered"]
            sb.node = g["som_node"]
            self.som_node = sb.node
            row_max = g["row_max"]

            pooled = None
            if sorted_pool:
                pooled = self.first_pointnet.forward_pooled(pn_in, g["ids_sorted"], row_max, M, epoch, need_dense=False, pos0=g["pos0"])
            elif train_pooled:
                pooled = self.first_pointnet.forward_pooled(pn_in, a.min_idx_i32, row_max, M, epoch,
                                                            need_dense=per_point or not _ops.POOLED_TRAIN_EPILOGUE)
            if pooled is not None:
                self.first_pn_out, self.first_pn_out_masked_max, _ = pooled
                if self._first_pn_out is None:
                    self._lazy["not_materialised"] = True
            else:
                self.first_pn_out = self.first_pointnet(pn_in, epoch)
                if self._first_pn_out is None:
                    self._lazy["first_p16"] = self.first_pointnet.last_p16
                    _, self.first_pn_out_masked_max = _ops.index_max_gather_p16(self.first_pointnet.last_p16, a.min_idx_i32, M, row_max)
                elif torch.is_grad_enabled() and self.first_pn_out.requires_grad:
                    gather_index = _ops.index_max(self.first_pn_out.detach(), a.min_idx_i32, M).long()
                    self.first_pn_out_masked_max = self.first_pn_out.gather(
                        dim=2, index=gather_index * row_max.unsqueeze(1).long())
                else:
                    _, self.first_pn_out_masked_max = _ops.index_max_gather(self.first_pn_out, a.min_idx_i32, M, row_max)

        if opt.som_k >= 2:
            self.knn_center_1, self.knn_feature_1 = self.knnlayer(self.som_node, self.first_pn_out_masked_max,
                                                                  node_knn_I, opt.som_k, opt.som_k_type, epoch)
            lead, feat = self.knn_center_1, self.knn_feature_1
        else:
            lead, feat = self.som_node, self.first_pn_out_masked_max
        forward_cat = getattr(self.final_pointnet, 'forward_cat', None)
        self.final_pn_out = (forward_cat(lead, feat, epoch) if forward_cat is not None
                             else self.final_pointnet(torch.cat((lead, feat), dim=1), epoch))
        if torch.is_grad_enabled() and self.final_pn_out.requires_grad:
            self.feature = _ops.lastdim_max_autograd(self.final_pn_out)
        else:
            self.feature = _ops.lastdim_max(self.final_pn_out.contiguous())
        if self.feature.dtype != torch.float32:
            self.feature = self.feature.float()
        return self.feature


class Classifier(_PlainAttrs, nn.Module):

    def __init__(self, opt):
        super().__init__()
        self.opt = opt
        self.feature_num = opt.feature_num
        kw = _bn_kwargs(opt)
        self.fc1 = MyLinear(self.feature_num, 512, activation=opt.activation, normalization=opt.normalization, **kw)
        self.fc2 = MyLinear(512, 256, activation=opt.activation, normalization=opt.normalization, **kw)
        self.fc3 = MyLinear(256, opt.classes, activation=None, normalization=None)
        self.dropout1 = nn.Dropout(p=opt.dropout)
        self.dropout2 = nn.Dropout(p=opt.dropout)

    @_head_inference
    def forward(self, feature, epoch=None):
        h = self.fc1(feature, epoch)
        if self.opt.dropout > 0.1:
            h = self.dropout1(h)
        self.fc2_out = self.fc2(h, epoch)
        if self.opt.dropout > 0.1:
            self.fc2_out = self.dropout2(self.fc2_out)
        return self.fc3(self.fc2_out, epoch)


class Segmenter(_PlainAttrs, nn.Module):

    def __init__(self, opt):
        super().__init__()
        _DENSE_HEADS.add(self)
        self.opt = opt
        self.feature_num = opt.feature_num
        c = 3 + 3 + 3 + 16 + 384 + 384 + self.feature_num * 2
        if opt.surface_normal:
            c += 3
        if opt.som_k >= 2:
# ... 323 lines not shown
```

so-net_amd/sonet_hip/_lib.py:

```python
import ctypes
import os

import torch

_HERE = os.path.dirname(os.path.abspath(__file__))
LIB_PATH = os.path.join(os.path.dirname(_HERE), "lib", "libsonet_hip.so")
VARIANTS_PATH = os.path.join(os.path.dirname(_HERE), "lib", "libsonet_hip_variants.so")
if os.environ.get("SONET_HIP_LIB"):
    LIB_PATH = os.environ["SONET_HIP_LIB"]

_vp = ctypes.c_void_p
_i = ctypes.c_int

SIGNATURES = {
    "sonet_abi_version": [],
    "sonet_build_arch": [],
    "sonet_last_error": [],
    "sonet_check_device": [],
    "sonet_range_log_set": [_vp],
    "sonet_pooled_wgrad_f32": [_vp, _vp, _vp, _i, _i, _i, _i, _i, _vp, _vp],
    "sonet_bn_running_update_f32": [_vp, _vp, _vp, _vp, ctypes.c_float, ctypes.c_float, _i, _vp],
    "sonet_knn_prepare_f32": [_vp, _vp, _i, _i, _i, _i, _vp, _vp, _vp, _vp],
    "sonet_pointmlp_h3_gather_f32": [_vp, _i, _i, _vp, _vp, _i, _vp, _vp, _vp, _i, _vp, _i, _i, _i, _vp],
    "sonet_planes_max_f32": [_vp, _vp, ctypes.c_longlong, _i, _i, _vp],
    "sonet_diag_mfma_f16_rate": [_i, _i, _vp, _vp, _vp],
    "sonet_index_max_f32": [_vp, _vp, _vp, _i, _i, _i, _i, _vp],
    "sonet_index_max_bf16": [_vp, _vp, _vp, _i, _i, _i, _i, _vp],
    "sonet_index_max_gather_f32": [_vp, _vp, _vp, _vp, _vp, _i, _i, _i, _i, _vp],
    "sonet_som_assign_f32": [_vp, _vp, _i, _i, _i, _i, _vp, _vp, _vp, _vp, _vp],
    "sonet_som_train_f32": [_vp, _vp, _i, _vp, _vp, _i, _i, _i, _i, _vp, _vp],
    "sonet_assemble_batch_f32": [_vp, ctypes.c_longlong, _vp, _i, _vp, _vp, _i, _i, _i, _i, _i, ctypes.c_longlong, ctypes.c_longlong,
                                 _vp, _vp, _vp, _vp, _vp, _vp, _vp, _vp, _vp, _vp],
    "sonet_som_assign_sort_ws_size": [_i, _i, _i, _i],
    "sonet_pointmlp_bf16_pool": [_vp, _i, _vp, _i, _vp, _vp, _vp, _i, _vp, _vp, _vp, _vp, _i, _i, _i, _i, _vp],
    "sonet_pointmlp_bf16_pool_xaff": [_vp, _i, _vp, _i, _vp, _vp, _vp, _i, _vp, _vp, _vp, _vp, _i, _i, _i, _i, _vp, _vp, _vp, _vp, _i, _vp],
    "sonet_pointmlp_h3_segpool_ws_size": [_i, _i, _i],
    "sonet_pointmlp_h3_segpool_f32": [_vp, _i, _vp, _i, _vp, _vp, _vp, _i, _vp, _vp, _vp, _i, _vp, _vp, _vp, _i, _i, _i, _vp, _vp, _vp, _vp, _i, _vp],
    "sonet_pointmlp_h3_stats_xaff_f32": [_vp, _i, _vp, _i, _vp, _vp, _vp, _i, _vp, _i, _i, _i, _vp, _vp, _vp, _vp, _vp, _vp, _vp, _i, _vp],
    "sonet_pointmlp_x3_bnb_f32": [_vp, _vp, _i, _vp, _vp, _vp, _vp, _vp, _vp, _vp, _vp, _i, _vp, _vp, _i, _i, _i, _vp, _vp, _vp, _i, _vp, _vp, _vp],
    "sonet_pointmlp_x3_bnb_acc_f32": [_vp, _vp, _i, _vp, _vp, _vp, _vp, _vp, _vp, _vp, _vp, _i, _vp, _vp, _vp, _i, _i, _i, _vp],
    "sonet_wgrad_x3_xaff_f32": [_vp, _vp, _vp, _vp, _i, _i, _i, _i, _vp, _vp, _i, _vp],
    "sonet_pooled_wgrad_xaff_f32": [_vp, _vp, _vp, _i, _i, _i, _i, _i, _vp, _vp, _vp, _i, _vp],
    "sonet_pack_multi": [_vp, _i, _i, _vp],
    "sonet_pack_multi_kc": [_i, _i],
    "sonet_bn_rider_set": [_vp, _vp, ctypes.c_float, ctypes.c_float, ctypes.c_float, _vp, _vp, _vp, _vp, _vp],
    "sonet_som_assign_sort_f32": [_vp, _vp, _vp, _i, _i, _i, _i, _vp, _vp, _vp, _vp, _vp, _vp, _vp, _vp, _vp, _vp, _vp, _vp],
    "sonet_som_assign_sort_det_f32": [_vp, _vp, _vp, _i, _i, _i, _i, _vp, _vp, _vp, _vp, _vp, _vp, _vp, _vp, _vp, _vp, _vp, _vp],
    "sonet_som_assign_sort_knn_f32": [_vp, _vp, _vp, _i, _i, _i, _i, _vp, _vp, _vp, _vp, _vp, _vp, _vp, _vp, _vp, _vp, _vp,
                                      _vp, _i, _i, _i, _vp, _vp, _vp, _vp],
    "sonet_som_group_f32": [_vp, _vp, _vp, _vp, _vp, _i, _i, _i, _i, _vp, _vp, _vp, _vp, _vp, _vp],
    "sonet_som_mask_i32": [_vp, _vp, _i, _i, _i, _vp],
    "sonet_node_gather_f32": [_vp, _vp, _vp, _i, _i, _i, _i, _vp],
    "sonet_knn_self_f32": [_vp, _vp, _i, _i, _i, _vp],
    "sonet_knn_group_f32": [_vp, _vp, _vp, _i, _i, _i, _i, _i, _vp, _vp, _vp],
    "sonet_lastdim_max_f32": [_vp, _vp, ctypes.c_longlong, _i, _vp],
    "sonet_knn_gather_f32": [_vp, _vp, _vp, _i, _i, _i, _i, _vp],
    "sonet_pointmlp_pack_size": [_i, _i],
    "sonet_pointmlp_pack_f32": [_vp, _vp, _i, _i, _vp],
    "sonet_pointmlp_f32": [_vp, _i, _vp, _i, _vp, _vp, _vp, _i, _vp, _i, _i, _i, _vp],
    "sonet_pointmlp_bf16_pack_size": [_i, _i],
    "sonet_pointmlp_bf16_pack": [_vp, _vp, _i, _i, _vp],
    "sonet_pointmlp_bf16": [_vp, _i, _vp, _i, _vp, _vp, _vp, _i, _vp, _i, _i, _i, _vp],
    "sonet_pointmlp_bf16_acc": [_vp, _i, _vp, _i, _vp, _vp, _vp, _i, _vp, _vp, _i, _i, _i, _vp],
    "sonet_pointmlp_bf16_bnb": [_vp, _vp, _i, _vp, _vp, _vp, _vp, _vp, _vp, _vp, _vp, _i, _vp, _vp, _vp, _i, _i, _i, _vp],
    "sonet_pointmlp_bf16_gather": [_vp, _i, _i, _vp, _vp, _i, _vp, _vp, _vp, _i, _vp, _i, _i, _i, _vp],
    "sonet_index_max_gather_bf16": [_vp, _vp, _vp, _vp, _vp, _i, _i, _i, _i, _vp],
    "sonet_index_max_gather_p16": [_vp, _vp, _vp, _vp, _vp, _i, _i, _i, _i, _vp],
    "sonet_node_gather_lead_affine_act_f32": [_vp, _vp, _vp, _vp, _vp, _vp, _i, _vp, _i, _i, _i, _i, _i, _vp],
    "sonet_node_gather_lead_affine_act_bf16": [_vp, _vp, _vp, _vp, _vp, _vp, _i, _vp, _i, _i, _i, _i, _i, _vp],
    "sonet_pointmlp_stats_ws_size": [_i, _i, _i],
    "sonet_pointmlp_h3_stats_f32": [_vp, _i, _vp, _i, _vp, _vp, _vp, _i, _vp, _i, _i, _i, _vp, _vp, _vp, _vp],
    "sonet_pointmlp_x3_stats_f32": [_vp, _i, _vp, _i, _vp, _vp, _vp, _i, _vp, _i, _i, _i, _vp, _vp, _vp, _vp],
    "sonet_pointmlp_bf16_stats_ws_size": [_i, _i, _i],
    "sonet_pointmlp_bf16_stats": [_vp, _i, _vp, _i, _vp, _vp, _vp, _i, _vp, _i, _i, _i, _vp, _vp, _vp, _vp],
    "sonet_pointmlp_bf16_stats_xaff": [_vp, _i, _vp, _i, _vp, _vp, _vp, _i, _vp, _i, _i, _i, _vp, _vp, _vp, _vp, _vp, _vp, _vp, _i, _vp],
    "sonet_pointmlp_h3_nodeadd_f32": [_vp, _i, _vp, _i, _vp, _vp, _vp, _i, _vp, _i, _i, _i, _vp, _vp, _i, _vp],
    "sonet_pointmlp_h3_nodeadd_stats_f32": [_vp, _i, _vp, _i, _vp, _vp, _vp, _i, _vp, _i, _i, _i, _vp, _vp, _i, _vp, _vp, _vp, _vp],
    "sonet_wgrad_x3_ws_size": [_i, _i, _i, _i],
    "sonet_wgrad_x3_f32": [_vp, _vp, _vp, _vp, _i, _i, _i, _i, _vp],
    "sonet_wgrad_bf16_ws_size": [_i, _i, _i, _i],
    "sonet_wgrad_bf16": [_vp, _vp, _vp, _vp, _i, _i, _i, _i, _vp],
    "sonet_wgrad_bf16_xaff": [_vp, _vp, _vp, _vp, _i, _i, _i, _i, _vp, _vp, _i, _vp],
    "sonet_pointmlp_x3_pack_size": [_i, _i],
    "sonet_pointmlp_x3_pack": [_vp, _vp, _i, _i, _vp],
    "sonet_pointmlp_x3_f32": [_vp, _i, _vp, _i, _vp, _vp, _vp, _i, _vp, _i, _i, _i, _vp],
    "sonet_pointmlp_h3_pack": [_vp, _vp, _i, _i, _vp],
    "sonet_pointmlp_h3_f32": [_vp, _i, _vp, _i, _vp, _vp, _vp, _i, _vp, _i, _i, _i, _vp],
    "sonet_lastdim_argmax_f32": [_vp, _vp, _vp, ctypes.c_longlong, _i, _vp],
    "sonet_lastdim_argmax_bf16": [_vp, _vp, _vp, ctypes.c_longlong, _i, _vp],
    "sonet_lastdim_max_bwd_f32": [_vp, _vp, _vp, ctypes.c_longlong, _i, _vp],
    "sonet_lastdim_max_bwd_bf16": [_vp, _vp, _vp, ctypes.c_longlong, _i, _vp],
    "sonet_knn_gather_bwd_ws_size": [_i, _i, _i],
    "sonet_knn_gather_bwd_f32": [_vp, _vp, _vp, _vp, _i, _i, _i, _i, _vp],
    "sonet_knn_gather_bwd_bf16": [_vp, _vp, _vp, _vp, _i, _i, _i, _i, _vp],
    "sonet_node_gather_bwd_ws_size": [_i, _i, _i],
    "sonet_node_gather_bwd_f32": [_vp, _vp, _vp, _vp, _i, _i, _i, _i, _vp],
    "sonet_node_gather_bwd_bf16": [_vp, _vp, _vp, _vp, _i, _i, _i, _i, _vp],
    "sonet_pointwise_bwd_apply_nodesum_ws_size": [_i, _i, _i],
    "sonet_pointwise_bwd_apply_nodesum_tile": [],
    "sonet_pointwise_bwd_apply_nodesum_f32": [_vp, _vp, _vp, _vp, _i, _vp, _vp, _vp, _vp, _i, _vp, _vp, _vp, _i, _i, _i, _vp],
    "sonet_p16_size": [_i, _i, _i],
    "sonet_p16_from_f32": [_vp, _vp, _i, _i, _i, _vp, _vp, _i, _vp],
    "sonet_p16_to_f32": [_vp, _vp, _i, _i, _i, _vp],
    "sonet_pointmlp_h3p_pack_size": [_i, _i],
    "sonet_pointmlp_h3p_pack": [_vp, _vp, _i, _i, _vp],
    "sonet_pointmlp_h3p_stats_ws_size": [_i, _i, _i],
    "sonet_pointmlp_h3p": [_vp, _i, _i, _vp, _vp, _i, _vp, _vp, _vp, _i, _vp, _vp, _i, _i, _i, _vp, _vp, _i, _vp, _vp, _vp, _vp],
    "sonet_pointresnet_bf16_pack_size": [],
    "sonet_pointresnet_bf16_pack": [_vp, _vp, _vp, _vp, _i, _vp, _vp],
    "sonet_pointresnet_bf16": [_vp, _i, _vp, _vp, _vp, _i, _i, _vp],
    "sonet_pointresnet_bf16_pool_ws_size": [_i, _i, _i],
    "sonet_pointresnet_bf16_pool": [_vp, _i, _vp, _vp, _vp, _vp, _vp, _vp, _vp, _vp, _i, _i, _i, _vp],
    "sonet_pointresnet_pack_size": [],
    "sonet_pointresnet_pack": [_vp, _vp, _vp, _vp, _i, _vp, _vp],
    "sonet_pointresnet_fused_f32": [_vp, _i, _vp, _vp, _vp, _i, _i, _vp],
    "sonet_pointresnet_fused_p16_f32": [_vp, _i, _vp, _vp, _vp, _vp, _i, _i, _vp],
    "sonet_pointresnet_pool_ws_size": [_i, _i, _i],
    "sonet_pointresnet_fused_pool_f32": [_vp, _i, _vp, _vp, _vp, _vp, _vp, _vp, _vp, _vp, _i, _i, _i, _vp],
    "sonet_pointresnet_fused_pool_p16_f32": [_vp, _i, _vp, _vp, _vp, _vp, _vp, _vp, _vp, _vp, _vp, _i, _i, _i, _vp],
    "sonet_knn_stage_columns": [_i, _i, _i],
    "sonet_knn_stage_prepare_f32": [_vp, _vp, _i, _i, _i, _i, _i, _vp, _vp, _vp, _vp],
    "sonet_knn_stage_input_p16": [_vp, _vp, _vp, _vp, _vp, _i, _i, _i, _i, _i, _vp, _vp],
    "sonet_pointmlp_h3p_gmax": [_vp, _i, _vp, _i, _vp, _vp, _vp, _i, _i, _i, _i, _i, _i, _i, _vp, _vp, _vp],
    "sonet_node_stage_columns": [_i, _i],
    "sonet_p16_flat_to_bcm_f32": [_vp, _vp, _i, _i, _i, _vp],
    "sonet_som_sort_group_f32": [_vp, _vp, _vp, _vp, _vp, _i, _i, _i, _i, _vp, _vp, _vp, _vp, _vp, _vp, _vp, _vp],
    "sonet_pointwise_bwd_stats_f32": [_vp, _vp, _vp, _vp, _i, _i, _i, _i, _vp, _vp],
    "sonet_pointwise_bwd_apply_f32": [_vp, _vp, _vp, _vp, _i, _vp, _vp, _vp, _vp, _i, _i, _i, _vp],
    "sonet_node_add_affine_act_f32": [_vp, _vp, _vp, _vp, _vp, _i, _i, _i, _i, _i, _vp],
    "sonet_linear_act_f32": [_vp, _vp, _vp, _vp, _i, _vp, _i, _i, _i, _vp],
    "sonet_pooled_dgrad_ws_size": [_i, _i, _i, _i],
    "sonet_pooled_wgrad_xbf16": [_vp, _vp, _vp, _i, _i, _i, _i, _i, _vp, _vp],
    "sonet_pooled_wgrad_xaff_xbf16": [_vp, _vp, _vp, _i, _i, _i, _i, _i, _vp, _vp, _vp, _i, _vp],
    "sonet_pooled_dgrad_obf16": [_vp, _vp, _vp, _i, _i, _i, _i, _i, _i, _vp, _vp, _vp, _vp],
    "sonet_pooled_dgrad_f32": [_vp, _vp, _vp, _i, _i, _i, _i, _i, _i, _vp, _vp, _vp, _vp],
    "sonet_pooled_dgrad_mfma_bf16": [_vp, _vp, _vp, _i, _i, _i, _i, _i, _i, _vp, _vp, _vp, _vp],
    "sonet_bn_fwd_coeffs_f32": [_vp, _vp, _vp, _vp, ctypes.c_float, _i, _vp, _vp, _vp, _vp],
    "sonet_bn_bwd_coeffs_f32": [_vp, _vp, _vp, _vp, ctypes.c_double, _i, _vp, _vp, _vp, _vp, _vp, _vp],
    "sonet_channel_affine_act_out_f32": [_vp, _vp, _vp, _i, _vp, _i, _i, _i, _vp],
    "sonet_chunk_mean_f32": [_vp, _vp, ctypes.c_longlong, _i, _i, _vp],
    "sonet_pointmlp_x3_pack_strided": [_vp, ctypes.c_longlong, ctypes.c_longlong, _vp, _i, _i, _i, _vp],
    "sonet_pointmlp_h3_pack_strided": [_vp, ctypes.c_longlong, ctypes.c_longlong, _vp, _i, _i, _i, _vp],
    "sonet_pointmlp_bf16_pack_strided": [_vp, ctypes.c_longlong, ctypes.c_longlong, _vp, _i, _i, _i, _vp],
    "sonet_adam_chunk": [],
    "sonet_fc_max_rows": [],
    "sonet_fc_bn_act_fwd_f32": [_vp, _vp, _vp, _vp, _vp, _vp, _vp, ctypes.c_float, ctypes.c_float, _i, _i, _i, _i, _vp, _vp, _vp, _vp],
    "sonet_fc_bn_act_bwd_f32": [_vp, _vp, _vp, _vp, _vp, _vp, _i, _i, _i, _i, _vp, _vp, _vp, _vp, _vp, _vp],
    "sonet_fc_dx_f32": [_vp, _vp, _i, _i, _i, _vp, _vp],
    "sonet_adam_multi_f32": [_vp, _vp, _vp, _vp, _vp, _vp, _i, ctypes.c_float, ctypes.c_float, ctypes.c_float, ctypes.c_float, ctypes.c_float, _vp],
    "sonet_channel_stats_f32": [_vp, _i, _i, _i, _vp, _vp, _vp, _vp],
    "sonet_channel_stats_bf16": [_vp, _i, _i, _i, _vp, _vp, _vp, _vp],
    "sonet_channel_affine_act_out_bf16": [_vp, _vp, _vp, _i, _vp, _i, _i, _i, _vp],
    "sonet_pointwise_bwd_stats_bf16": [_vp, _vp, _vp, _vp, _i, _i, _i, _i, _vp, _vp],
    "sonet_pointwise_bwd_apply_bf16": [_vp, _vp, _vp, _vp, _i, _vp, _vp, _vp, _vp, _i, _i, _i, _vp],
    "sonet_channel_affine_act_f32": [_vp, _vp, _vp, _i, _i, _i, _i, _vp],
    "sonet_chamfer_nn_f32": [_vp, _vp, _vp, _i, _i, _i, _vp],
    "sonet_chamfer_loss_ws_size": [_i, _i, _i],
    "sonet_chamfer_loss_f32": [_vp, _vp, _vp, _vp, _vp, _vp, _vp, _vp, _i, _i, _i, _vp],
    "sonet_chamfer_grad_f32": [_vp, _vp, _vp, _vp, _vp, _vp, _vp, _vp, _vp, _i, _i, _i, _vp],
    "sonet_upconv3x3_pack_size": [_i, _i],
    "sonet_upconv3x3_pack_f32": [_vp, _vp, _i, _i, _vp],
    "sonet_upconv3x3_f32": [_vp, _vp, _vp, _vp, _i, _vp, _i, _i, _i, _i, _i, _vp, _vp],
    "sonet_upconv3x3_dgrad_pack_size": [_i, _i],
    "sonet_upconv3x3_dgrad_pack_f32": [_vp, _vp, _i, _i, _vp],
    "sonet_upconv3x3_dgrad_f32": [_vp, _vp, _vp, _i, _i, _i, _i, _i, _vp],
    "sonet_upconv3x3_wgrad_ws_size": [_i, _i, _i, _i, _i],
    "sonet_upconv3x3_wgrad_f32": [_vp, _vp, _vp, _vp, _i, _i, _i, _i, _i, _vp],
    "sonet_seg_metrics_ws_size": [_i, _i, _i],
    "sonet_seg_metrics_f32": [_vp, _vp, _vp, _vp, _i, _vp, _vp, _vp, _vp, _vp, _vp, _vp, _vp, _vp, _i, _i, _i, _vp],
    "sonet_retrieval_chunk_keys": [],
    "sonet_retrieval_ws_size": [_i, _i, _i, _i],
    "sonet_retrieval_lists_f32": [_vp, _vp, _vp, _vp, _i, _i, _vp, _vp, _vp, _vp, _vp, _vp, _vp, _i, _i, _i, _vp],
}
_RESTYPES = {
    "sonet_build_arch": ctypes.c_char_p,
    "sonet_last_error": ctypes.c_char_p,
    "sonet_pointmlp_pack_size": ctypes.c_size_t,
    "sonet_pointmlp_stats_ws_size": ctypes.c_size_t,
    "sonet_pointmlp_h3_segpool_ws_size": ctypes.c_size_t,
    "sonet_pointmlp_bf16_stats_ws_size": ctypes.c_size_t,
    "sonet_wgrad_x3_ws_size": ctypes.c_size_t,
    "sonet_wgrad_bf16_ws_size": ctypes.c_size_t,
    "sonet_pointmlp_x3_pack_size": ctypes.c_size_t,
    "sonet_p16_size": ctypes.c_size_t,
    "sonet_knn_stage_columns": ctypes.c_size_t,
    "sonet_node_stage_columns": ctypes.c_size_t,
    "sonet_knn_gather_bwd_ws_size": ctypes.c_size_t,
    "sonet_node_gather_bwd_ws_size": ctypes.c_size_t,
    "sonet_pointwise_bwd_apply_nodesum_ws_size": ctypes.c_size_t,
    "sonet_pointmlp_h3p_pack_size": ctypes.c_size_t,
    "sonet_pointmlp_h3p_stats_ws_size": ctypes.c_size_t,
    "sonet_pointmlp_bf16_pack_size": ctypes.c_size_t,
    "sonet_pointresnet_pack_size": ctypes.c_size_t,
    "sonet_pointresnet_bf16_pack_size": ctypes.c_size_t,
    "sonet_pointresnet_bf16_pool_ws_size": ctypes.c_size_t,
    "sonet_pointresnet_pool_ws_size": ctypes.c_size_t,
    "sonet_pooled_dgrad_ws_size": ctypes.c_size_t,
    "sonet_pooled_dgrad_tail_ws_size": ctypes.c_size_t,
    "sonet_som_assign_sort_ws_size": ctypes.c_size_t,
    "sonet_chamfer_nn2_ws_size": ctypes.c_size_t,
    "sonet_chamfer_loss_ws_size": ctypes.c_size_t,
    "sonet_upconv3x3_pack_size": ctypes.c_size_t,
    "sonet_upconv3x3_dgrad_pack_size": ctypes.c_size_t,
    "sonet_upconv3x3_wgrad_ws_size": ctypes.c_size_t,
    "sonet_seg_metrics_ws_size": ctypes.c_size_t,
    "sonet_retrieval_ws_size": ctypes.c_size_t,
}

VARIANT_SIGNATURES = {
    "sonet_chamfer_nn2_ws_size": [_i, _i, _i],
    "sonet_chamfer_nn2_f32": [_vp, _vp, _vp, _vp, _vp, _i, _i, _i, _vp],
    "sonet_pointmlp_h3_kmax_f32": [_vp, _i, _vp, _i, _vp, _vp, _vp, _i, _vp, _vp, _i, _i, _i, _i, _vp],
    "sonet_pooled_dgrad_tail_ws_size": [_i, _i, _i],
    "sonet_pooled_dgrad_tail_f32": [_vp, _vp, _vp, _i, _i, _i, _i, _i, _i, _vp, _vp, _vp, _vp, _vp, _vp, _vp, _vp, _i, _vp, _vp, _vp],
}

_lib = None


class SonetHipError(RuntimeError):
    pass


def load():
    global _lib
    if _lib is not None:
        return _lib
    if not os.path.exists(LIB_PATH):
        raise SonetHipError(
            "libsonet_hip.so is not built (%s).  Build it with `make -C so-net_amd/csrc` or "
            "`python -c 'import __graft_entry__ as g; g.build()'`.  There is no CPU fallback." % LIB_PATH)
    try:
        lib = ctypes.CDLL(LIB_PATH)
    except OSError as e:
        raise SonetHipError("cannot load %s: %s" % (LIB_PATH, e))
    for name, args in SIGNATURES.items():
        fn = getattr(lib, name)
        fn.argtypes = args
        fn.restype = _RESTYPES.get(name, ctypes.c_int)
    for name, args in VARIANT_SIGNATURES.items():
        fn = getattr(lib, name, None)
        if fn is not None:
            fn.argtypes = args
            fn.restype = _RESTYPES.get(name, ctypes.c_int)
    _lib = lib
    return lib


def last_error():
    return load().sonet_last_error().decode("utf-8", "replace")


def check(status, what=""):
    if status != 0:
        raise SonetHipError("%s failed (status %d): %s" % (what or "libsonet_hip", status, last_error()))


_device_ok = {}


def require_device(device):
    if device.index in _device_ok:
        return
    if device.type != "cuda" and torch.cuda.is_available():
        raise SonetHipError("sonet_hip needs its tensors on an MI355X (gfx950) GPU, got one on %s; there is no CPU fallback" % device)
    if not torch.cuda.is_available():
        raise SonetHipError("sonet_hip needs an MI355X (gfx950) GPU; torch.cuda.is_available() is False "
                            "and there is no CPU fallback")
    idx = device.index if device.index is not None else torch.cuda.current_device()
    ok = _device_ok.get(idx)
    if ok is None:
        with torch.cuda.device(idx):
            check(load().sonet_check_device(), "sonet_check_device")
        _device_ok[idx] = True


# ... 21 lines not shown
```

so-net_amd/sonet_hip/ops.py:

```python
import numpy as np
import torch

from . import _lib
from ._lib import SonetHipError, check, ptr, stream_ptr
import functools as _functools
import threading as _threading

_tls = _threading.local()
_join_lock = _threading.Lock()


def _consumes_rider(fn):
    @_functools.wraps(fn)
    def wrapped(*a, **k):
        try:
            return fn(*a, **k)
        finally:
            _rider_done()
    return wrapped


_TIMING = None


# ... 590 lines not shown
def assemble_batch(src, offsets, nodes_src, idx, N, K, flags, seed, step, replay_idx=None, replay_draws=None, want_draws=False,
                   sizes=None):
    _chk(src, "src", torch.float32, 2)
    _chk(offsets, "offsets", torch.int64, 1)
    _chk(nodes_src, "nodes_src", torch.float32, 3)
    _chk(idx, "idx", torch.int64, 1)
    S, M = nodes_src.shape[0], nodes_src.shape[1]
    B, N, K, flags = idx.shape[0], int(N), int(K), int(flags)
    if src.shape[0] != 6 or nodes_src.shape[2] != 3 or offsets.shape[0] != S + 1:
        raise SonetHipError("src must be 6 x P, nodes_src S x M x 3 and offsets S+1, got %s, %s, %s"
                            % (tuple(src.shape), tuple(nodes_src.shape), tuple(offsets.shape)))
    if B < 1 or N < 1 or not 1 <= K <= min(M, BATCH_MAX_K):
        raise SonetHipError("need B >= 1, N >= 1 and 1 <= K <= min(M, %d), got B=%d N=%d K=%d M=%d" % (BATCH_MAX_K, B, N, K, M))
    if sizes is not None:
        ii, sizes = idx.cpu().numpy(), np.asarray(sizes)
        if ii.min() < 0 or ii.max() >= S:
            raise SonetHipError("idx out of range [0, %d): min %d max %d" % (S, ii.min(), ii.max()))
        smallest = int(sizes[ii].min())
        if not flags & BATCH_SHAPENET and smallest < N:
            raise SonetHipError("N=%d > n_s=%d points of a cloud in the batch (modelnet / shrec sample without replacement)" % (N, smallest))
    dev = _same_device(src, offsets, nodes_src, idx, replay_idx, replay_draws)
    D = batch_draw_size(N, M)
    if replay_idx is not None:
        _chk(replay_idx, "replay_idx", torch.int64)
        if tuple(replay_idx.shape) != (B, N):
            raise SonetHipError("replay_idx must be B x N = %s, got %s" % ((B, N), tuple(replay_idx.shape)))
    if replay_draws is not None:
        _chk(replay_draws, "replay_draws", torch.float64)
        if tuple(replay_draws.shape) != (B, D):
            raise SonetHipError("replay_draws must be B x D = %s, got %s" % ((B, D), tuple(replay_draws.shape)))
    f32 = dict(dtype=torch.float32, device=dev)
    r = dict(pc=torch.empty((B, 3, N), **f32), sn=torch.empty((B, 3, N), **f32), node=torch.empty((B, 3, M), **f32),
             chosen=torch.empty((B, N), dtype=torch.int64, device=dev), knn_I=torch.empty((B, M, K), dtype=torch.int64, device=dev),
             bad=torch.empty((B,), dtype=torch.int32, device=dev))
    if want_draws:
        r["draws"] = torch.zeros((B, D), dtype=torch.float64, device=dev)
    with _lib.on_device(dev), _timed("assemble_batch"):
        check(_lib.load().sonet_assemble_batch_f32(
            ptr(src), src.shape[1], ptr(offsets), S, ptr(nodes_src), ptr(idx), B, N, M, K, flags, _i64(seed), _i64(step), ptr(replay_idx) if replay_idx is not None else None,
            ptr(replay_draws) if replay_draws is not None else None, ptr(r["draws"]) if want_draws else None,
            ptr(r["pc"]), ptr(r["sn"]), ptr(r["node"]), ptr(r["chosen"]), ptr(r["knn_I"]), ptr(r["bad"]), stream_ptr()),
            "sonet_assemble_batch_f32")
    return r


def knn_group(coord, feat, knn_I, center_avg):
    _chk(coord, "coord", torch.float32, 3)
    _chk(feat, "feat", torch.float32, 3)
    _chk(knn_I, "knn_I", torch.int64, 3)
    dev = _same_device(coord, feat, knn_I)
    B, C, M = feat.shape
    K = knn_I.shape[2]
    center = torch.empty((B, 3, M), dtype=torch.float32, device=dev)
    out = torch.empty((B, 3 + C, M, K), dtype=torch.float32, device=dev)
    with _lib.on_device(dev), _timed("knn_group"):
        check(_lib.load().sonet_knn_group_f32(ptr(coord), ptr(feat), ptr(knn_I), B, C, M, K, int(bool(center_avg)), ptr(center), ptr(out),
                                              stream_ptr()), "sonet_knn_group_f32")
    return center, out


def lastdim_max(x):
    if x.dtype == torch.bfloat16:
        x = x.float()
    if not x.is_contiguous() or x.dtype != torch.float32:
        raise SonetHipError("lastdim_max needs a contiguous float32 tensor")
    dev = _same_device(x)
    K = x.shape[-1]
    out = torch.empty(x.shape[:-1], dtype=torch.float32, device=dev)
    if out.numel() == 0:
        return out
    with _lib.on_device(dev), _timed("lastdim_max"):
        check(_lib.load().sonet_lastdim_max_f32(ptr(x), ptr(out), out.numel(), K, stream_ptr()), "sonet_lastdim_max_f32")
    return out


def knn_gather(x, knn_I):
    _chk(x, "som_node", torch.float32, 3)
    _chk(knn_I, "som_node_knn_I", torch.int64, 3)
    B, C, M = x.shape
    if knn_I.shape[0] != B or knn_I.shape[1] != M:
        raise SonetHipError("knn_I must be B x M x K, got %s for x %s" % (tuple(knn_I.shape), tuple(x.shape)))
    K = knn_I.shape[2]
    dev = _same_device(x, knn_I)
    out = torch.empty((B, C, M, K), dtype=torch.float32, device=dev)
    with _lib.on_device(dev), _timed("knn_gather"):
        check(_lib.load().sonet_knn_gather_f32(ptr(x), ptr(knn_I), ptr(out), B, C, M, K, stream_ptr()), "sonet_knn_gather_f32")
    return out


def knn_gather_bwd(g, knn_I, M):
    if g.dtype not in (torch.float32, torch.bfloat16):
        raise SonetHipError("knn_gather_bwd: f32 or bf16 gradient")
    _chk(g, "g", g.dtype, 4)
    _chk(knn_I, "som_node_knn_I", torch.int64, 3)
    B, C, Mq, K = g.shape
    if tuple(knn_I.shape) != (B, Mq, K) or Mq != M:
        raise SonetHipError("knn_gather_bwd: knn_I must be B x M x K with the M of the gathered tensor")
    dev = _same_device(g, knn_I)
    lib = _lib.load()
    gx = torch.empty((B, C, M), dtype=torch.float32, device=dev)
    ws = torch.empty((lib.sonet_knn_gather_bwd_ws_size(B, M, K),), dtype=torch.uint8, device=dev)
    fn = lib.sonet_knn_gather_bwd_bf16 if g.dtype == torch.bfloat16 else lib.sonet_knn_gather_bwd_f32
    with _lib.on_device(dev), _timed("knn_gather_bwd"):
        check(fn(ptr(g), ptr(knn_I), ptr(gx), ptr(ws), B, C, M, K, stream_ptr()), "sonet_knn_gather_bwd")
    return gx


class _LastDimMax(torch.autograd.Function):

    @staticmethod
    def forward(ctx, x):
        xc = x.contiguous()
        K = xc.shape[-1]
        rows = xc.numel() // K
        out = torch.empty(xc.shape[:-1], dtype=xc.dtype, device=xc.device)
        idx = torch.empty(xc.shape[:-1], dtype=torch.int32, device=xc.device)
        lib = _lib.load()
        fn = lib.sonet_lastdim_argmax_bf16 if xc.dtype == torch.bfloat16 else lib.sonet_lastdim_argmax_f32
        with _lib.on_device(xc.device), _timed("lastdim_argmax"):
            check(fn(ptr(xc), ptr(out), ptr(idx), rows, K, stream_ptr()), "sonet_lastdim_argmax")
        ctx.save_for_backward(idx)
        ctx.K = K
        return out

    @staticmethod
    def backward(ctx, g):
        (idx,) = ctx.saved_tensors
        gc = g.contiguous()
        gx = torch.empty(tuple(gc.shape) + (ctx.K,), dtype=gc.dtype, device=gc.device)
        lib = _lib.load()
        fn = lib.sonet_lastdim_max_bwd_bf16 if gc.dtype == torch.bfloat16 else lib.sonet_lastdim_max_bwd_f32
        with _lib.on_device(gc.device), _timed("lastdim_max_bwd"):
            check(fn(ptr(gc), ptr(idx), ptr(gx), gc.numel(), ctx.K, stream_ptr()), "sonet_lastdim_max_bwd")
        return gx


def lastdim_max_autograd(x):
    if not x.is_cuda or x.dtype not in (torch.float32, torch.bfloat16) or x.numel() == 0:
        return torch.max(x, dim=-1)[0]
    return _LastDimMax.apply(x)


import os as _os

POINTMLP_PRECISION = _os.environ.get("SONET_POINTMLP_PRECISION", "h3")


FUSE_POINTRESNET = _os.environ.get("SONET_FUSE_POINTRESNET", "1") != "0"
FUSE_POOL = _os.environ.get("SONET_FUSE_POOL", "1") != "0"
GATHER_NODE_STAGE = _os.environ.get("SONET_GATHER_NODE_STAGE", "1") != "0"
NODE_LINEAR_SPLIT = _os.environ.get("SONET_NODE_LINEAR_SPLIT", "1") != "0"
P16_CHAINS = _os.environ.get("SONET_P16_CHAINS", "1") != "0"
NODE_STAGE_P16 = _os.environ.get("SONET_NODE_STAGE_P16", "1") != "0"
POOLED_TRAIN_EPILOGUE = _os.environ.get("SONET_POOLED_TRAIN_EPILOGUE", "1") != "0"
H3_SEGPOOL = _os.environ.get("SONET_H3_SEGPOOL", "1") != "0"
H3_NORM_ON_LOAD = _os.environ.get("SONET_H3_NORM_ON_LOAD", "1") != "0"
TRAIN_ASSIGN_SORT = _os.environ.get("SONET_TRAIN_ASSIGN_SORT", "1") != "0"
WGRAD_KERNEL = _os.environ.get("SONET_WGRAD_KERNEL", "1") != "0"


RANGE_GUARD = _os.environ.get("SONET_RANGE_GUARD", "1") != "0"
_RANGE_SLOTS = 32
_B_2047, _B_65504, _B_XLOW, _B_WLOW, _B_WLOW32 = 0x44FFE000, 0x477FE000, 0x3E800000, 0x3B800000, 0x3E000000
_range_logs = {}
_range_active = None
_range_ptr_set = False


def _bits_to_float(u):
    import struct
    return struct.unpack("<f", struct.pack("<I", int(u) & 0xFFFFFFFF))[0]


class range_scope:

    def __init__(self, device, private=False):
        self.device = torch.device(device)
        self.names = []
        self.enabled = RANGE_GUARD and self.device.type == "cuda"
        self.log = None
        self._prev = None
        self._own = torch.zeros((_RANGE_SLOTS * 8,), dtype=torch.int32, device=self.device) if (private and self.enabled) else None

    def __enter__(self):
        global _range_active
        self._prev = _range_active
        if self.enabled:
            idx = self.device.index if self.device.index is not None else torch.cuda.current_device()
            log = self._own if self._own is not None else _range_logs.get(idx)
            if log is None:
                log = torch.zeros((_RANGE_SLOTS * 8,), dtype=torch.int32, device=self.device)
                _range_logs[idx] = log
            else:
                log.zero_()
            self.log = log
            _range_active = self
        return self

    def __exit__(self, *exc):
        global _range_active
        _range_active = self._prev
        _range_unset()
        return False

    def _slot(self, name):
        i = min(len(self.names), _RANGE_SLOTS - 1)
        self.names.append(name)
        return self.log.data_ptr() + i * 32

    def violations(self):
        if not self.enabled or not self.names:
            return []
        w = self.log.cpu().view(_RANGE_SLOTS, 8).tolist()
        shared = {}
        out = []
        for n, name in enumerate(self.names):
            i = min(n, _RANGE_SLOTS - 1)
            if i in shared:
                continue
            shared[i] = True
            x, wt, hid = (v & 0xFFFFFFFF for v in w[i][:3])
            low_ok = n < _RANGE_SLOTS - 1
            if x > _B_2047:
                out.append((name, "max |x| = %g exceeds 2047" % _bits_to_float(x)))
            elif low_ok and 0 < x < _B_XLOW:
                out.append((name, "max |x| = %g is below %g (fp16 residuals go subnormal)" % (_bits_to_float(x), _bits_to_float(_B_XLOW))))
            if name.startswith("pointresnet_fused"):
                if wt > _B_65504:
                    out.append((name, "max |w| = %g exceeds %g" % (_bits_to_float(wt) / 32.0, 65504.0 / 32.0)))
                elif low_ok and 0 < wt < _B_WLOW32:
                    out.append((name, "max |w| = %g is below 2^-8" % (_bits_to_float(wt) / 32.0)))
            elif name.startswith("pointmlph3p") or name.startswith("upconv3x3"):
                if wt > _B_2047:
                    out.append((name, "max |w| = %g exceeds 2047" % _bits_to_float(wt)))
                elif low_ok and 0 < wt < _B_WLOW:
                    out.append((name, "max |w| = %g is below 2^-8" % _bits_to_float(wt)))
            elif wt > _B_65504:
                out.append((name, "max |w| = %g exceeds 65504" % _bits_to_float(wt)))
            elif low_ok and 0 < wt < _B_WLOW:
                out.append((name, "max |w| = %g is below 2^-8" % _bits_to_float(wt)))
            if hid > _B_2047:
                out.append((name, "a hidden activation reaches %g > 2047" % _bits_to_float(hid)))
        return out


_range_warned = False
_range_pending = []


def range_warn(bad):
    global _range_warned
    if not _range_warned:
        import warnings
        warnings.warn("sonet_hip: fp16-split (h3) operand range left by %d launch(es), e.g. %s: %s -- recomputing in the "
                      "range-safe x3 arithmetic (SONET_POINTMLP_PRECISION=x3 selects it from the start)"
                      % (len(bad), bad[0][0], bad[0][1]), RuntimeWarning, stacklevel=3)
        _range_warned = True


def _range_defer(scope):
    if not scope.enabled or not scope.names or torch.cuda.is_current_stream_capturing():
        return
    host = torch.empty((_RANGE_SLOTS * 8,), dtype=torch.int32, pin_memory=True)
    host.copy_(scope.log, non_blocking=True)
    ev = torch.cuda.Event()
    ev.record()
    _range_pending.append((ev, host, list(scope.names)))


range_scope.defer = _range_defer


def range_deferred_check():
    global POINTMLP_PRECISION
    while _range_pending and _range_pending[0][0].query():
        _, host, names = _range_pending.pop(0)
        probe = range_scope.__new__(range_scope)
        probe.enabled, probe.names, probe.log = True, names, host
        bad = probe.violations()
        if bad:
            range_warn(bad)
            POINTMLP_PRECISION = "x3"
            _range_pending.clear()
            return bad
    return []


def run_guarded(call, device, can_rerun):
    device = torch.device(device)
    if POINTMLP_PRECISION != "h3" or not RANGE_GUARD or device.type != "cuda" or _range_active is not None:
        return call()
    if not can_rerun:
        range_deferred_check()
        if POINTMLP_PRECISION != "h3":
            return call()
        with range_scope(device) as rs:
            out = call()
        rs.defer()
        return out
    with range_scope(device) as rs:
        out = call()
    if torch.cuda.is_current_stream_capturing():
        return out
    bad = rs.violations()
    if bad:
        range_warn(bad)
# ... 680 lines not shown
        with _lib.on_device(p.device), _timed("p16_to_f32"):
            check(_lib.load().sonet_p16_to_f32(ptr(p.data), ptr(x), p.B, p.C, p.L, stream_ptr()), "sonet_p16_to_f32")
    return x


def pointmlp_h3p_pack(weight2d):
    _chk(weight2d, "weight", torch.float32, 2)
    dev = _same_device(weight2d)
    Cout, Cin = weight2d.shape
    lib = _lib.load()
    with _lib.on_device(dev):
        wp = torch.empty((lib.sonet_pointmlp_h3p_pack_size(Cin, Cout) // 4,), dtype=torch.int32, device=dev)
        check(lib.sonet_pointmlp_h3p_pack(ptr(weight2d), ptr(wp), Cin, Cout, stream_ptr()), "sonet_pointmlp_h3p_pack")
    return wp


@_consumes_rider
def pointmlp_h3p(x1, wp, scale, shift, relu, Cout, x2=None, out="f32", gidx=None, z=None, zidx=None, stats=False, tag=None):
    if not isinstance(x1, P16) or (x2 is not None and not isinstance(x2, P16)):
        raise SonetHipError("pointmlp_h3p: P16 inputs (ops.p16_from_f32)")
    if wp.dtype != torch.int32:
        raise SonetHipError("pointmlp_h3p: an h3p pack (ops.pointmlp_h3p_pack)")
    B, C1, L1 = x1.shape
    L = L1
    if gidx is not None:
        _chk(gidx, "gidx", torch.int32, 2)
        if gidx.shape[0] != B:
            raise SonetHipError("pointmlp_h3p: gidx must have B rows")
        L = gidx.shape[1]
    C2 = 0
    if x2 is not None:
        if x2.B != B or x2.L != L:
            raise SonetHipError("x2 must be B x C2 x L")
        C2 = x2.C
        if C1 % 16 != 0:
            raise SonetHipError("pointmlp_h3p: with a second input C1 must be a multiple of 16")
    _chk(scale, "scale", torch.float32, 1)
    _chk(shift, "shift", torch.float32, 1)
    if (z is None) != (zidx is None):
        raise SonetHipError("pointmlp_h3p: z and zidx come together")
    ZM = 0
    if z is not None:
        _chk(z, "z", torch.float32, 3)
        _chk(zidx, "zidx", torch.int32, 2)
        if tuple(z.shape[:2]) != (B, Cout) or tuple(zidx.shape) != (B, L):
            raise SonetHipError("pointmlp_h3p: z must be B x Cout x M and zidx B x L")
        ZM = z.shape[2]
    if out not in ("f32", "p16", "both") or (stats and out != "f32"):
        raise SonetHipError("pointmlp_h3p: out is 'f32', 'p16' or 'both' (statistics: 'f32')")
    dev = _same_device(x1.data, x2.data if x2 is not None else None, wp, scale, shift, gidx, z, zidx)
    lib = _lib.load()
    cin_pack = (C1 + C2) if C2 else C1
    if wp.numel() * 4 != lib.sonet_pointmlp_h3p_pack_size(cin_pack, Cout):
        raise SonetHipError("packed weight has %d bytes, expected %d for Cin=%d Cout=%d"
                            % (wp.numel() * 4, lib.sonet_pointmlp_h3p_pack_size(cin_pack, Cout), cin_pack, Cout))
    y = torch.empty((B, Cout, L), dtype=torch.float32, device=dev) if out in ("f32", "both") else None
    yp = p16_empty(B, Cout, L, dev) if out in ("p16", "both") else None
    mean = var = ws = None
    if stats:
        mean = torch.empty((Cout,), dtype=torch.float32, device=dev)
        var = torch.empty((Cout,), dtype=torch.float32, device=dev)
        ws = torch.empty((lib.sonet_pointmlp_h3p_stats_ws_size(B, Cout, L),), dtype=torch.uint8, device=dev)
    if B * L * Cout != 0:
        name = "pointmlph3p%s_%dx%d_L%d" % ("_nodeadd" if z is not None else "_stats" if stats else ("_" + tag) if tag else "", C1 + C2, Cout, L)
        _range_arm(name)
        with _lib.on_device(dev), _timed(name):
            check(lib.sonet_pointmlp_h3p(ptr(x1.data), C1, L1, ptr(gidx), ptr(x2.data) if x2 is not None else None, C2, ptr(wp), ptr(scale), ptr(shift),
                                         int(bool(relu)), ptr(y), ptr(yp.data) if yp is not None else None, B, Cout, L, ptr(z), ptr(zidx), ZM,
                                         ptr(ws), ptr(mean), ptr(var), stream_ptr()), "sonet_pointmlp_h3p")
    if stats:
        return y, mean, var
    return y if out == "f32" else yp if out == "p16" else (y, yp)


def node_stage_columns(B, M):
    return (B * M + 127) // 128 * 128


def p16_flat(C, L, nvalid, device):
    if nvalid == L:
        return p16_empty(1, C, L, device)
    n = _lib.load().sonet_p16_size(1, C, L)
    return P16(torch.zeros((n,), dtype=torch.uint8, device=device), 1, C, L)


def pointmlp_h3p_gmax(x1, wp, scale, shift, relu, Cout, GK, G, ngout, x2=None, out="p16", Lout=None):
    if not isinstance(x1, P16) or (x2 is not None and not isinstance(x2, P16)):
        raise SonetHipError("pointmlp_h3p_gmax: P16 inputs")
    if wp.dtype != torch.int32:
        raise SonetHipError("pointmlp_h3p_gmax: an h3p pack (ops.pointmlp_h3p_pack)")
    if x1.B != 1 or (x2 is not None and (x2.B != 1 or x2.L != x1.L)):
        raise SonetHipError("pointmlp_h3p_gmax: one flat cloud (B == 1), x2 with the columns of x1")
    if out not in ("p16", "f32"):
        raise SonetHipError("pointmlp_h3p_gmax: out is 'p16' or 'f32'")
    C1, L = x1.C, x1.L
    C2 = x2.C if x2 is not None else 0
    _chk(scale, "scale", torch.float32, 1)
    _chk(shift, "shift", torch.float32, 1)
    dev = _same_device(x1.data, x2.data if x2 is not None else None, wp, scale, shift)
    lib = _lib.load()
    if wp.numel() * 4 != lib.sonet_pointmlp_h3p_pack_size(C1 + C2, Cout):
        raise SonetHipError("packed weight has %d bytes, expected %d for Cin=%d Cout=%d"
                            % (wp.numel() * 4, lib.sonet_pointmlp_h3p_pack_size(C1 + C2, Cout), C1 + C2, Cout))
    Lout = int(ngout if Lout is None else Lout)
    y = torch.empty((ngout, Cout), dtype=torch.float32, device=dev) if out == "f32" else None
    yp = p16_flat(Cout, Lout, ngout, dev) if out == "p16" else None
    name = "pointmlph3p_gmax%d_%dx%d_L%d" % (GK, C1 + C2, Cout, int(ngout) * int(GK))
    _range_arm(name)
    with _lib.on_device(dev), _timed(name):
        check(lib.sonet_pointmlp_h3p_gmax(ptr(x1.data), C1, ptr(x2.data) if x2 is not None else None, C2, ptr(wp), ptr(scale), ptr(shift),
                                          int(bool(relu)), Cout, L, int(GK), int(G), int(ngout), Lout, ptr(y), ptr(yp.data) if yp is not None else None,
                                          stream_ptr()), "sonet_pointmlp_h3p_gmax")
    return y if out == "f32" else yp


def knn_stage_prepare(coord, knn_I, K, center_avg):
    _chk(coord, "coord", torch.float32, 3)
    _chk(knn_I, "knn_I", torch.int64, 3)
    B, three, M = coord.shape
    KI = knn_I.shape[2]
    if three != 3 or tuple(knn_I.shape[:2]) != (B, M) or KI < K or not 1 <= K <= 128:
        raise SonetHipError("knn_stage_prepare: coord B x 3 x M, knn_I B x M x (>= K), 1 <= K <= 128")
    dev = _same_device(coord, knn_I)
    lib = _lib.load()
    Lm = node_stage_columns(B, M)
    Lp = int(lib.sonet_knn_stage_columns(B, M, int(K)))
    center = torch.empty((B, 3, M), dtype=torch.float32, device=dev)
    cp = p16_flat(3, Lm, B * M, dev)
    rec = torch.empty((Lp, 4), dtype=torch.int32, device=dev)
    _range_arm("knn_stage_prepare")
    with _lib.on_device(dev), _timed("knn_stage_prepare"):
        check(lib.sonet_knn_stage_prepare_f32(ptr(coord), ptr(knn_I), KI, int(bool(center_avg)), B, M, int(K), ptr(center), ptr(cp.data), ptr(rec),
                                              stream_ptr()), "sonet_knn_stage_prepare_f32")
    return dict(center=center, center_p16=cp, rec=rec, B=B, M=M, K=int(K), G=min(16, 128 // int(K)), Lp=Lp)


def knn_stage_input(prep, z, wl, scale, shift, relu):
    if not isinstance(z, P16) or z.B != 1 or z.L != node_stage_columns(prep["B"], prep["M"]):
        raise SonetHipError("knn_stage_input: z is a P16 1 x C x Lm activation")
    _chk(wl, "wl", torch.float32, 2)
    _chk(scale, "scale", torch.float32, 1)
    _chk(shift, "shift", torch.float32, 1)
    C = z.C
    if tuple(wl.shape) != (C, 3) or scale.numel() != C or shift.numel() != C:
        raise SonetHipError("knn_stage_input: wl C x 3, scale / shift C")
    dev = _same_device(prep["rec"], z.data, wl, scale, shift)
    h1 = p16_empty(1, C, prep["Lp"], dev)
    name = "knn_stage_input_%dx%d" % (C, prep["B"] * prep["M"] * prep["K"])
    _range_arm(name)
    with _lib.on_device(dev), _timed(name):
        check(_lib.load().sonet_knn_stage_input_p16(ptr(prep["rec"]), ptr(z.data), ptr(wl), ptr(scale), ptr(shift), int(bool(relu)),
                                                    prep["B"], prep["M"], prep["K"], C, ptr(h1.data), stream_ptr()), "sonet_knn_stage_input_p16")
    return h1


def p16_flat_to_bcm(p, B, M):
    if p.B != 1 or p.L != node_stage_columns(B, M):
        raise SonetHipError("p16_flat_to_bcm: a 1 x C x (B M) activation")
    x = torch.empty((B, p.C, M), dtype=torch.float32, device=p.device)
    with _lib.on_device(p.device), _timed("p16_flat_to_bcm"):
        check(_lib.load().sonet_p16_flat_to_bcm_f32(ptr(p.data), ptr(x), B, p.C, M, stream_ptr()), "sonet_p16_flat_to_bcm_f32")
    return x


def pointresnet_pack(w1, w2, w3, w4):
    for i, w in enumerate((w1, w2, w3, w4)):
        _chk(w, "w%d" % (i + 1), torch.float32, 2)
    if (w1.shape[0], tuple(w2.shape), tuple(w3.shape), tuple(w4.shape)) != (64, (128, 64), (256, 128), (384, 320)) or w1.shape[1] > 16:
        raise SonetHipError("pointresnet_fused supports Cin0<=16 -> 64 -> 128 -> 256 -> [320] -> 384 only")
    dev = _same_device(w1, w2, w3, w4)
    lib = _lib.load()
    ws = torch.empty((lib.sonet_pointresnet_pack_size(),), dtype=torch.uint8, device=dev)
    with _lib.on_device(dev):
        check(lib.sonet_pointresnet_pack(ptr(w1), ptr(w2), ptr(w3), ptr(w4), w1.shape[1], ptr(ws), stream_ptr()),
              "sonet_pointresnet_pack")
    return ws


def pointresnet_fused(x, wstream, affine, want_p16=False):
    _chk_member(wstream, "wstream", torch.uint8, (_lib.load().sonet_pointresnet_pack_size(),))
    _chk(x, "x", torch.float32, 3)
    _chk(affine, "affine", torch.float32, 2)
    if tuple(affine.shape) != (832, 2):
        raise SonetHipError("affine must be 832 x 2 (scale, shift)")
    dev = _same_device(x, wstream, affine)
    B, Cin0, L = x.shape
    only = want_p16 == "only"
    y = None if only else torch.empty((B, 384, L), dtype=torch.float32, device=dev)
    yp = p16_empty(B, 384, L, dev) if want_p16 else None
    if B * L == 0:
        return (y, yp) if want_p16 else y
    _range_arm("pointresnet_fused_L%d" % L)
    with _lib.on_device(dev), _timed("pointresnet_fused%s_L%d" % ("_p16only" if only else "_p16" if want_p16 else "", L)):
        if want_p16:
            check(_lib.load().sonet_pointresnet_fused_p16_f32(ptr(x), Cin0, ptr(wstream), ptr(affine), ptr(y), ptr(yp.data), B, L, stream_ptr()),
                  "sonet_pointresnet_fused_p16_f32")
        else:
            check(_lib.load().sonet_pointresnet_fused_f32(ptr(x), Cin0, ptr(wstream), ptr(affine), ptr(y), B, L, stream_ptr()),
                  "sonet_pointresnet_fused_f32")
    return (y, yp) if want_p16 else y


def pointresnet_fused_pool(sg, wstream, affine, M, want_p16=False):
    x_sorted = sg["x_aug_sorted"]
    _chk_sort_group(sg, M)
    _chk_member(wstream, "wstream", torch.uint8, (_lib.load().sonet_pointresnet_pack_size(),))
    _chk(x_sorted, "x_sorted", torch.float32, 3)
    _chk(affine, "affine", torch.float32, 2)
    if tuple(affine.shape) != (832, 2):
        raise SonetHipError("affine must be 832 x 2 (scale, shift)")
    dev = _same_device(x_sorted, wstream, affine, sg["ids_sorted"], sg["pos0"], sg["node_off"], sg["count"])
    B, Cin0, L = x_sorted.shape
    lib = _lib.load()
    ws = torch.empty((lib.sonet_pointresnet_pool_ws_size(B, L, int(M)),), dtype=torch.uint8, device=dev)
    out = torch.empty((B, 384, int(M)), dtype=torch.float32, device=dev)
    outp = p16_flat(384, node_stage_columns(B, int(M)), B * int(M), dev) if want_p16 else None
    _range_arm("pointresnet_fused_pool_L%d" % L)
    with _lib.on_device(dev), _timed("pointresnet_fused_pool_L%d" % L):
        if want_p16:
            check(lib.sonet_pointresnet_fused_pool_p16_f32(ptr(x_sorted), Cin0, ptr(wstream), ptr(affine), ptr(sg["ids_sorted"]), ptr(sg["pos0"]),
                                                           ptr(sg["node_off"]), ptr(sg["count"]), ptr(ws), ptr(out), ptr(outp.data), B, L, int(M),
                                                           stream_ptr()), "sonet_pointresnet_fused_pool_p16_f32")
        else:
            check(lib.sonet_pointresnet_fused_pool_f32(ptr(x_sorted), Cin0, ptr(wstream), ptr(affine), ptr(sg["ids_sorted"]), ptr(sg["pos0"]),
                                                       ptr(sg["node_off"]), ptr(sg["count"]), ptr(ws), ptr(out), B, L, int(M), stream_ptr()),
                  "sonet_pointresnet_fused_pool_f32")
    return (out, outp) if want_p16 else out


def pointresnet_bf16_pack(w1, w2, w3, w4):
    for i, w in enumerate((w1, w2, w3, w4)):
        _chk(w, "w%d" % (i + 1), torch.float32, 2)
    if (w1.shape[0], tuple(w2.shape), tuple(w3.shape), tuple(w4.shape)) != (64, (128, 64), (256, 128), (384, 320)) or w1.shape[1] > 16:
        raise SonetHipError("pointresnet_bf16 supports Cin0<=16 -> 64 -> 128 -> 256 -> [320] -> 384 only")
    dev = _same_device(w1, w2, w3, w4)
    lib = _lib.load()
    ws = torch.empty((lib.sonet_pointresnet_bf16_pack_size(),), dtype=torch.uint8, device=dev)
    with _lib.on_device(dev):
        check(lib.sonet_pointresnet_bf16_pack(ptr(w1), ptr(w2), ptr(w3), ptr(w4), w1.shape[1], ptr(ws), stream_ptr()),
              "sonet_pointresnet_bf16_pack")
    return ws


def pointresnet_bf16(x, wstream, affine):
    _chk_member(wstream, "wstream", torch.uint8, (_lib.load().sonet_pointresnet_bf16_pack_size(),))
    _chk(x, "x", torch.float32, 3)
    _chk(affine, "affine", torch.float32, 2)
    if tuple(affine.shape) != (832, 2):
        raise SonetHipError("affine must be 832 x 2 (scale, shift)")
    dev = _same_device(x, wstream, affine)
    B, Cin0, L = x.shape
    y = torch.empty((B, 384, L), dtype=torch.bfloat16, device=dev)
    if y.numel() == 0:
        return y
    with _lib.on_device(dev), _timed("pointresnet_bf16_L%d" % L):
        check(_lib.load().sonet_pointresnet_bf16(ptr(x), Cin0, ptr(wstream), ptr(affine), ptr(y), B, L, stream_ptr()),
              "sonet_pointresnet_bf16")
    return y


def pointresnet_bf16_pool(sg, wstream, affine, M):
    x_sorted = sg["x_aug_sorted"]
    _chk_sort_group(sg, M)
    _chk_member(wstream, "wstream", torch.uint8, (_lib.load().sonet_pointresnet_bf16_pack_size(),))
    _chk(x_sorted, "x_sorted", torch.float32, 3)
    _chk(affine, "affine", torch.float32, 2)
    if tuple(affine.shape) != (832, 2):
        raise SonetHipError("affine must be 832 x 2 (scale, shift)")
    dev = _same_device(x_sorted, wstream, affine, sg["ids_sorted"], sg["pos0"], sg["node_off"], sg["count"])
    B, Cin0, L = x_sorted.shape
    lib = _lib.load()
    ws = torch.empty((lib.sonet_pointresnet_bf16_pool_ws_size(B, L, int(M)),), dtype=torch.uint8, device=dev)
    out = torch.empty((B, 384, int(M)), dtype=torch.float32, device=dev)
    with _lib.on_device(dev), _timed("pointresnet_bf16_pool_L%d" % L):
        check(lib.sonet_pointresnet_bf16_pool(ptr(x_sorted), Cin0, ptr(wstream), ptr(affine), ptr(sg["ids_sorted"]), ptr(sg["pos0"]),
                                              ptr(sg["node_off"]), ptr(sg["count"]), ptr(ws), ptr(out), B, L, int(M), stream_ptr()),
              "sonet_pointresnet_bf16_pool")
    return out


@_consumes_rider
def channel_stats(y):
    _chk(y, "y", dim=3)
    if y.dtype not in (torch.float32, torch.bfloat16):
        raise SonetHipError("channel_stats: float32 or bfloat16, got %s" % y.dtype)
    dev = _same_device(y)
    B, C, L = y.shape
    ws = torch.empty((2 * C,), dtype=torch.float64, device=dev)
    mean = torch.empty((C,), dtype=torch.float32, device=dev)
    var = torch.empty((C,), dtype=torch.float32, device=dev)
    lib = _lib.load()
    fn = lib.sonet_channel_stats_f32 if y.dtype == torch.float32 else lib.sonet_channel_stats_bf16
    try:
        with _lib.on_device(dev), _timed("channel_stats" if y.dtype == torch.float32 else "channel_stats_bf16"):
            check(fn(ptr(y), B, C, L, ptr(ws), ptr(mean), ptr(var), stream_ptr()), "sonet_channel_stats")
    finally:
        _rider_done()
    return mean, var


def channel_affine_act_(y, scale, shift, relu):
    _chk(y, "y", torch.float32, 3)
    B, C, L = y.shape
    _chk_cvec(C, scale=scale, shift=shift)
    dev = _same_device(y, scale, shift)
    with _lib.on_device(dev), _timed("channel_affine_act"):
# ... 743 lines not shown
```

Baseline: 76420.

## Fuse kNN stage-input build into layer-2 h3p GEMM with group max

Measured after the change: 78050 (median of 6 runs). 1.02x the previous value.

```diff
diff --git a/include/sonet_hip.h b/include/sonet_hip.h
--- a/include/sonet_hip.h
+++ b/include/sonet_hip.h
@@ -136,6 +136,9 @@
                               int B, int M, int K, int C, void *h1_p16, sonet_stream_t stream);
 int sonet_pointmlp_h3p_gmax(const void *x1p, int C1, const void *x2p, int C2, const void *Wp, const float *scale, const float *shift,
                             int relu, int Cout, int L, int GK, int G, int ngout, int Lout, float *y, void *yp, sonet_stream_t stream);
+int sonet_knn_layer2_gmax_p16(const void *rec, const void *z_p16, const float *wl, const float *scale1, const float *shift1, int relu1,
+                              int B, int M, int K, int Cin, const void *Wp, const float *scale2, const float *shift2, int relu2,
+                              int Cout, int GK, int G, int ngout, int Lout, void *yp, sonet_stream_t stream);
 int sonet_p16_flat_to_bcm_f32(const void *p16, float *x, int B, int C, int M, sonet_stream_t stream);
 
 int sonet_lastdim_argmax_f32(const float *x, float *out, int32_t *idx, long long rows, int K, sonet_stream_t stream);
diff --git a/so-net_amd/csrc/device.hpp b/so-net_amd/csrc/device.hpp
--- a/so-net_amd/csrc/device.hpp
+++ b/so-net_amd/csrc/device.hpp
@@ -111,6 +111,18 @@
 __device__ __forceinline__ float clamp_keep_nan(float w, float lim) { return w < -lim ? -lim : (w > lim ? lim : w); }
 __device__ __forceinline__ int p16_channel(int h, int e) { return 4 * h + (e & 3) + 8 * (e >> 2); }
 
+constexpr int GM_STRIDE = 136;
+__device__ __forceinline__ float nan_max(float m, float v) { return (v > m || v != v) ? v : m; }
+__device__ __forceinline__ void gmax_p16_store(float m0, float m1, float split_lo, RangeAcc &yr, void *yp, int chunk, int h2, int p,
+                                               size_t Lout, size_t n_out) {
+    range_track(yr, m0, m1);
+    unsigned hv, mv;
+    p16_split2(__builtin_amdgcn_fmed3f(m0, split_lo * 32.f, 65504.f), __builtin_amdgcn_fmed3f(m1, split_lo * 32.f, 65504.f), hv, mv);
+    unsigned *dst = reinterpret_cast<unsigned *>(static_cast<char *>(yp) + ((((size_t)chunk * 2) * 2 + h2) * Lout + n_out) * 16) + p;
+    dst[0] = hv;
+    dst[Lout * 8] = mv;
+}
+
 __device__ __forceinline__ void split3_pair(float x0, float x1, unsigned &h, unsigned &m, unsigned &l) {
     h = cvt_pk_bf16(x0, x1);
     const float r0 = x0 - __uint_as_float(h << 16), r1 = x1 - __uint_as_float(h & 0xFFFF0000u);
diff --git a/so-net_amd/csrc/knn_h1.hpp b/so-net_amd/csrc/knn_h1.hpp
--- /dev/null
+++ b/so-net_amd/csrc/knn_h1.hpp
@@ -0,0 +1,69 @@
+#pragma once
+
+__device__ __forceinline__ float knn_h1_coef(int kind, bool in, int c, const float *__restrict__ wl, const float *__restrict__ scale,
+                                             const float *__restrict__ shift) {
+    if (!in) return 0.f;
+    return kind < 3 ? 32.f * wl[c * 3 + kind] : kind == 3 ? scale[c] : 32.f * shift[c];
+}
+
+struct KnnCol {
+    f32x2_t d0, d1, d2;
+    bool valid, ok;
+};
+__device__ __forceinline__ KnnCol knn_col(const int4 r) {
+    KnnCol k;
+    k.d0 = f32x2_t{__int_as_float(r.y), __int_as_float(r.y)};
+    k.d1 = f32x2_t{__int_as_float(r.z), __int_as_float(r.z)};
+    k.d2 = f32x2_t{__int_as_float(r.w), __int_as_float(r.w)};
+    k.valid = r.x != -2;
+    k.ok = r.x >= 0;
+    return k;
+}
+
+template <typename V>
+__device__ __forceinline__ V knn_h1_preact(V z32, V w0, V w1, V w2, V sc, V sh, V d0, V d1, V d2) {
+    V a = __builtin_elementwise_fma(w0, d0, z32);
+    a = __builtin_elementwise_fma(w1, d1, a);
+    a = __builtin_elementwise_fma(w2, d2, a);
+    return __builtin_elementwise_fma(a, sc, sh);
+}
+
+template <bool PACKED>
+__device__ __forceinline__ void knn_h1_pair(unsigned zh, unsigned zm, const float *const (&cf)[5], const KnnCol &k, float lo, RangeAcc &xr,
+                                            unsigned &hv, unsigned &mv) {
+    const f32x2_t w0 = *reinterpret_cast<const f32x2_t *>(cf[0]), w1 = *reinterpret_cast<const f32x2_t *>(cf[1]),
+                w2 = *reinterpret_cast<const f32x2_t *>(cf[2]), sc = *reinterpret_cast<const f32x2_t *>(cf[3]),
+                sh = *reinterpret_cast<const f32x2_t *>(cf[4]);
+    const f16x2_t zh2 = __builtin_bit_cast(f16x2_t, zh), zm2 = __builtin_bit_cast(f16x2_t, zm);
+    f32x2_t a;
+    if constexpr (PACKED) {
+        a = knn_h1_preact<f32x2_t>(__builtin_convertvector(zh2, f32x2_t) + __builtin_convertvector(zm2, f32x2_t), w0, w1, w2, sc, sh, k.d0, k.d1, k.d2);
+    } else {
+#pragma unroll
+        for (int e = 0; e < 2; ++e)
+            a[e] = knn_h1_preact<float>((float)zh2[e] + (float)zm2[e], w0[e], w1[e], w2[e], sc[e], sh[e], k.d0[e], k.d1[e], k.d2[e]);
+    }
+    if (!k.valid) a = f32x2_t{0.f, 0.f};
+    range_track(xr, a[0], a[1]);
+    p16_split2(__builtin_amdgcn_fmed3f(a[0], lo, 65504.f), __builtin_amdgcn_fmed3f(a[1], lo, 65504.f), hv, mv);
+}
+
+__device__ __forceinline__ void knn_h1_half(const uint4 zhq, const uint4 zmq, const float *const (&cf)[5], const KnnCol &k, float lo,
+                                            RangeAcc &xr, uint4 &hq, uint4 &mq) {
+    const unsigned zh[4] = {zhq.x, zhq.y, zhq.z, zhq.w}, zm[4] = {zmq.x, zmq.y, zmq.z, zmq.w};
+    unsigned hv[4], mv[4];
+#pragma unroll
+    for (int q = 0; q < 4; ++q) {
+        const float *const cq[5] = {cf[0] + 2 * q, cf[1] + 2 * q, cf[2] + 2 * q, cf[3] + 2 * q, cf[4] + 2 * q};
+        knn_h1_pair<true>(zh[q], zm[q], cq, k, lo, xr, hv[q], mv[q]);
+    }
+    hq = make_uint4(hv[0], hv[1], hv[2], hv[3]);
+    mq = make_uint4(mv[0], mv[1], mv[2], mv[3]);
+}
+
+__device__ __forceinline__ unsigned range_act_bits(const RangeAcc &r, int relu) {
+    if (!relu) return range_amax_bits(r);
+    const unsigned pos = r.mp > 0 ? (unsigned)r.mp : 0u, nan_neg = r.mn > 0xFF800000u ? (r.mn & 0x7FFFFFFFu) : 0u;
+    return pos > nan_neg ? pos : nan_neg;
+}
+__device__ __forceinline__ unsigned range_x32_out(unsigned bits) { return bits > (5u << 23) ? bits - (5u << 23) : 0u; }
diff --git a/so-net_amd/csrc/knn_layer.hip b/so-net_amd/csrc/knn_layer.hip
--- /dev/null
+++ b/so-net_amd/csrc/knn_layer.hip
@@ -0,0 +1,296 @@
+#include "common.hpp"
+#include "knn_h1.hpp"
+
+namespace {
+
+constexpr int KL_STAGE = 8;
+constexpr int KL_MAXC = 512;
+constexpr int KL_WRING = 4;
+
+struct KnnLayerArgs {
+    const int4 *rec;
+    const uint4 *zp;
+    const float *wl, *scale1, *shift1;
+    const uint4 *Wp;
+    const float *scale2, *shift2;
+    char *yp;
+    unsigned *rlog;
+    long long Lm;
+    int relu1, relu2, KC, NS, KCP, CT, Cout, GK, G, ngout, Lout;
+    int abl;
+};
+
+struct KnnLayerLds {
+    uint4 x[2][KL_STAGE][2][2][128];
+    float coef[5][KL_MAXC];
+    float aff[KL_MAXC / 32][2][2][16];
+    unsigned wmax[4];
+};
+static_assert(sizeof(KnnLayerLds) <= 160 * 1024, "LDS of a CU");
+static_assert(4 * 32 * GM_STRIDE * sizeof(float) <= sizeof(uint4) * 2 * KL_STAGE * 2 * 2 * 128, "the epilogue's staging fits the operand buffers");
+
+template <int MT>
+__global__ __launch_bounds__(256) void knn_layer2_gmax_kernel(const KnnLayerArgs a)
+{
+    __shared__ __attribute__((aligned(16))) KnnLayerLds lds;
+    const int tid = (int)threadIdx.x;
+    const int lane = tid & 63, wave = __builtin_amdgcn_readfirstlane(tid >> 6);
+    const int j = lane & 31, h = lane >> 5;
+    const int blk = (int)blockIdx.x;
+    const int col = tid & 127, hh = __builtin_amdgcn_readfirstlane(tid >> 7);
+    const int4 rcol = a.rec[(long long)blk * 128 + col];
+    const KnnCol kcol = knn_col(rcol);
+    const int KC = a.KC, Cin = KC * 16;
+
+    for (int t = tid; t < KL_MAXC; t += 256) {
+        const int c = (t >> 4) * 16 + p16_channel((t >> 3) & 1, t & 7);
+#pragma unroll
+        for (int kind = 0; kind < 5; ++kind) lds.coef[kind][t] = knn_h1_coef(kind, c < Cin, c, a.wl, a.scale1, a.shift1);
+    }
+    for (int o = tid; o < a.Cout; o += 256) {
+        const int rr = o & 31;
+        float *t = &lds.aff[o >> 5][(rr >> 2) & 1][0][(rr & 3) | ((rr >> 3) << 2)];
+        t[0] = a.scale2[o] * (32.f / 1024.f);
+        t[16] = a.shift2[o] * 32.f;
+    }
+
+    RangeAcc xr = {0, 0u};
+    const float lo1 = a.relu1 ? 0.f : -65504.f;
+    const uint4 *zbase = a.zp + (long long)hh * a.Lm + (kcol.ok ? rcol.x : 0);
+
+    uint4 Zh[2], Zm[2];
+    unsigned hv4[4], mv4[4];
+    f32x2_t creg[2][5];
+    auto load_coef = [&](f32x2_t (&c)[5], int kc, int u) {
+        const int ci = (kc < KC ? kc : KC - 1) * 16 + hh * 8 + 2 * u;
+#pragma unroll
+        for (int kind = 0; kind < 5; ++kind) c[kind] = *reinterpret_cast<const f32x2_t *>(&lds.coef[kind][ci]);
+    };
+    auto gather = [&](int slot, int kc) {
+        kc = kc < KC ? kc : KC - 1;
+        const uint4 *zq = zbase + (long long)kc * 4 * a.Lm;
+#ifdef SONET_VARIANTS
+        if (a.abl & 2) zq = a.zp + (long long)hh * a.Lm;
+#endif
+        Zh[slot] = zq[0];
+        Zm[slot] = zq[2 * a.Lm];
+    };
+    auto build_unit = [&](int slot, const f32x2_t (&c)[5], int kc, int buf, int q, int u) {
+        const bool in = kc < KC, live = kcol.ok && in;
+        const float *const cf[5] = {reinterpret_cast<const float *>(&c[0]), reinterpret_cast<const float *>(&c[1]), reinterpret_cast<const float *>(&c[2]),
+                                    reinterpret_cast<const float *>(&c[3]), reinterpret_cast<const float *>(&c[4])};
+        KnnCol kk = kcol;
+        kk.valid = kcol.valid && in;
+        const unsigned zh = u == 0 ? Zh[slot].x : u == 1 ? Zh[slot].y : u == 2 ? Zh[slot].z : Zh[slot].w;
+        const unsigned zm = u == 0 ? Zm[slot].x : u == 1 ? Zm[slot].y : u == 2 ? Zm[slot].z : Zm[slot].w;
+        knn_h1_pair<false>(live ? zh : 0u, live ? zm : 0u, cf, kk, lo1, xr, hv4[u], mv4[u]);
+        if (u == 3) {
+            lds.x[buf][q][0][hh][col] = make_uint4(hv4[0], hv4[1], hv4[2], hv4[3]);
+            lds.x[buf][q][1][hh][col] = make_uint4(mv4[0], mv4[1], mv4[2], mv4[3]);
+        }
+    };
+
+    const int NS = a.NS, KCT = NS * KL_STAGE;
+    const uint4 *wbase = a.Wp + ((size_t)(wave * MT) * a.KCP * 2) * 64 + lane;
+    uint4 Wr[KL_WRING][2];
+    auto load_w = [&](int kc0, int t) {
+        int kc = kc0 + t / MT;
+        kc = kc < KCT ? kc : KCT - 1;
+        const uint4 *wq = wbase + ((size_t)(t % MT) * a.KCP + kc) * 128;
+#ifdef SONET_VARIANTS
+        if (a.abl & 1) wq = wbase;
+#endif
+        Wr[t % KL_WRING][0] = wq[0];
+        Wr[t % KL_WRING][1] = wq[64];
+    };
+
+    f32x16 acc[MT][4];
+#pragma unroll
+    for (int mt = 0; mt < MT; ++mt)
+#pragma unroll
+        for (int c = 0; c < 4; ++c)
+#pragma unroll
+            for (int r = 0; r < 16; ++r) acc[mt][c][r] = 0.f;
+
+    f16x8 Bf[2][2][4];
+    auto read_b = [&](int set, int buf, int q) {
+#pragma unroll
+        for (int c = 0; c < 4; ++c) {
+            Bf[set][0][c] = __builtin_bit_cast(f16x8, lds.x[buf][q][0][h][32 * c + j]);
+            Bf[set][1][c] = __builtin_bit_cast(f16x8, lds.x[buf][q][1][h][32 * c + j]);
+        }
+    };
+
+#pragma unroll
+    for (int t = 0; t < KL_WRING - 1; ++t) load_w(0, t);
+    {
+        uint4 Ph[KL_STAGE], Pm[KL_STAGE];
+#pragma unroll
+        for (int q = 0; q < KL_STAGE; ++q) {
+            gather(0, q);
+            Ph[q] = Zh[0];
+            Pm[q] = Zm[0];
+        }
+        __syncthreads();
+#pragma unroll
+        for (int q = 0; q < KL_STAGE; ++q) {
+            Zh[0] = Ph[q];
+            Zm[0] = Pm[q];
+            f32x2_t c4[4][5];
+#pragma unroll
+            for (int u = 0; u < 4; ++u) load_coef(c4[u], q, u);
+#pragma unroll
+            for (int u = 0; u < 4; ++u) build_unit(0, c4[u], q, 0, q, u);
+        }
+    }
+    if (NS > 1) load_coef(creg[0], KL_STAGE, 0);
+
+    auto stage = [&](int s, auto build_next) {
+        constexpr bool BUILD = decltype(build_next)::value;
+        const int buf = s & 1, kc0 = s * KL_STAGE, kn = kc0 + KL_STAGE;
+        __syncthreads();
+        read_b(0, buf, 0);
+        if constexpr (BUILD) gather(0, kn);
+#pragma unroll
+        for (int q = 0; q < KL_STAGE; ++q) {
+#pragma unroll
+            for (int mt = 0; mt < MT; ++mt) {
+                const int t = q * MT + mt;
+                load_w(kc0, t + KL_WRING - 1);
+                if (mt == 0 && q + 1 < KL_STAGE) {
+                    read_b((q + 1) & 1, buf, q + 1);
+                    if constexpr (BUILD) gather((q + 1) & 1, kn + q + 1);
+                }
+                const f16x8 wh = __builtin_bit_cast(f16x8, Wr[t % KL_WRING][0]), wm = __builtin_bit_cast(f16x8, Wr[t % KL_WRING][1]);
+#pragma unroll
+                for (int term = 0; term < 3; ++term)
+#pragma unroll
+                    for (int c = 0; c < 4; ++c)
+                        acc[mt][c] = __builtin_amdgcn_mfma_f32_32x32x16_f16(term == 0 ? wm : wh, Bf[q & 1][term == 1 ? 1 : 0][c], acc[mt][c], 0, 0, 0);
+#pragma unroll
+                for (int u = 0; u < 4; ++u)
+                    if (BUILD && u * MT / 4 == mt) {
+                        const int n = q * 4 + u;
+                        load_coef(creg[(n + 1) & 1], kn + (n + 1) / 4, (n + 1) % 4);
+                        build_unit(q & 1, creg[n & 1], kn + q, buf ^ 1, q, u);
+                    }
+#define KL_GAP2 __builtin_amdgcn_sched_group_barrier(0x008, 1, 0); __builtin_amdgcn_sched_group_barrier(0x002, 3, 0); \
+                __builtin_amdgcn_sched_group_barrier(0x008, 1, 0); __builtin_amdgcn_sched_group_barrier(0x002, 4, 0);
+                KL_GAP2 KL_GAP2 KL_GAP2 KL_GAP2 KL_GAP2 KL_GAP2
+#undef KL_GAP2
+                __builtin_amdgcn_sched_barrier(0);
+            }
+        }
+    };
+    for (int s = 0; s + 1 < NS; ++s) stage(s, bool_c<true>{});
+    stage(NS - 1, bool_c<false>{});
+    __syncthreads();
+
+    float (*gm)[GM_STRIDE] = reinterpret_cast<float (*)[GM_STRIDE]>(reinterpret_cast<char *>(&lds.x[0][0][0][0][0]) + (size_t)wave * (32 * GM_STRIDE * 4));
+    RangeAcc yr = {0, 0u};
+    const float relu_thr = a.relu2 ? 0.f : -__builtin_inff();
+    const float split_lo = a.relu2 ? 0.f : -2047.f;
+    int tid2 = tid;
+    asm volatile("" : "+v"(tid2));
+    const int je = tid2 & 31, he = (tid2 >> 5) & 1;
+    const int p = tid2 & 3, g = (tid2 & 63) >> 2;
+    const long long n_out = (long long)blk * a.G + g;
+    const bool node = g < a.G && n_out < a.ngout;
+    const float *rbase = &gm[2 * (p & 1) + 8 * (p >> 1)][(g < a.G ? g : 0) * a.GK];
+#pragma unroll
+    for (int mt = 0; mt < MT; ++mt) {
+        const int ct = wave * MT + mt;
+        float sc16[16], sh16[16];
+        {
+            const float4 *t4 = reinterpret_cast<const float4 *>(&lds.aff[ct][he][0][0]);
+#pragma unroll
+            for (int u = 0; u < 4; ++u) {
+                const float4 s4 = t4[u], h4 = t4[4 + u];
+                sc16[4 * u] = s4.x; sc16[4 * u + 1] = s4.y; sc16[4 * u + 2] = s4.z; sc16[4 * u + 3] = s4.w;
+                sh16[4 * u] = h4.x; sh16[4 * u + 1] = h4.y; sh16[4 * u + 2] = h4.z; sh16[4 * u + 3] = h4.w;
+            }
+        }
+#pragma unroll
+        for (int c = 0; c < 4; ++c)
+#pragma unroll
+            for (int r = 0; r < 16; ++r) {
+                const float v = __fmaf_rn(acc[mt][c][r], sc16[r], sh16[r]);
+                gm[(r & 3) + 8 * (r >> 2) + 4 * he][32 * c + je] = v < relu_thr ? 0.f : v;
+            }
+        __builtin_amdgcn_fence(__ATOMIC_RELEASE, "wavefront");
+        __builtin_amdgcn_wave_barrier();
+        __builtin_amdgcn_fence(__ATOMIC_ACQUIRE, "wavefront");
+        float m0[4], m1[4];
+#pragma unroll
+        for (int qh = 0; qh < 4; ++qh) {
+            const float *r0 = rbase + (16 * (qh >> 1) + 4 * (qh & 1)) * GM_STRIDE;
+            m0[qh] = r0[0];
+            m1[qh] = r0[GM_STRIDE];
+        }
+        for (int k = 1; k < a.GK; ++k) {
+#pragma unroll
+            for (int qh = 0; qh < 4; ++qh) {
+                const float *r0 = rbase + (16 * (qh >> 1) + 4 * (qh & 1)) * GM_STRIDE;
+                m0[qh] = nan_max(m0[qh], r0[k]);
+                m1[qh] = nan_max(m1[qh], r0[GM_STRIDE + k]);
+            }
+        }
+        if (node) {
+#pragma unroll
+            for (int qh = 0; qh < 4; ++qh) {
+                const int qq = qh >> 1, h2 = qh & 1;
+                gmax_p16_store(m0[qh], m1[qh], split_lo, yr, a.yp, ct * 2 + qq, h2, p, (size_t)a.Lout, (size_t)n_out);
+            }
+        }
+        __builtin_amdgcn_fence(__ATOMIC_RELEASE, "wavefront");
+        __builtin_amdgcn_wave_barrier();
+        __builtin_amdgcn_fence(__ATOMIC_ACQUIRE, "wavefront");
+    }
+
+    if (a.rlog != nullptr) {
+        const unsigned b1 = range_x32_out(wave_umax(range_act_bits(xr, a.relu1)));
+        const unsigned b2 = range_x32_out(wave_umax(range_act_bits(yr, a.relu2)));
+        if ((tid2 & 63) == 0) lds.wmax[wave] = b1 > b2 ? b1 : b2;
+        __syncthreads();
+        if (tid2 == 0) {
+            const unsigned m01 = lds.wmax[0] > lds.wmax[1] ? lds.wmax[0] : lds.wmax[1], m23 = lds.wmax[2] > lds.wmax[3] ? lds.wmax[2] : lds.wmax[3];
+            const unsigned mx = m01 > m23 ? m01 : m23;
+            if (mx > __atomic_load_n(a.rlog + 2, __ATOMIC_RELAXED)) atomicMax(a.rlog + 2, mx);
+            if (blk == 0) atomicMax(a.rlog + 1, reinterpret_cast<const unsigned *>(a.Wp + (size_t)a.CT * a.KCP * 128)[0]);
+        }
+    }
+}
+
+}
+
+extern "C" int sonet_knn_layer2_gmax_p16(const void *rec, const void *z_p16, const float *wl, const float *scale1, const float *shift1, int relu1,
+                                         int B, int M, int K, int Cin, const void *Wp, const float *scale2, const float *shift2, int relu2,
+                                         int Cout, int GK, int G, int ngout, int Lout, void *yp, sonet_stream_t stream)
+{
+    const char *what = "sonet_knn_layer2_gmax_p16";
+    SONET_REQUIRE(rec && z_p16 && wl && scale1 && shift1 && Wp && scale2 && shift2 && yp, "%s: NULL pointer", what);
+    SONET_REQUIRE(B > 0 && M > 0 && Cin > 0 && Cout > 0 && K >= 1 && K <= 128, "%s: bad size B=%d M=%d Cin=%d Cout=%d K=%d", what, B, M, Cin, Cout, K);
+    SONET_REQUIRE(GK == K && G == knn_stage_groups(K) && (long long)ngout == (long long)B * M, "%s: the grouping of the K-level layout is GK=%d G=%d ngout=%d", what,
+                  K, knn_stage_groups(K), B * M);
+    SONET_REQUIRE(Lout >= ngout, "%s: Lout=%d (the planes' column count) below ngout=%d", what, Lout, ngout);
+    if (Cout % 128 != 0 || Cout > KL_MAXC) return sonet::fail(SONET_ERR_UNSUPPORTED, "%s: Cout=%d must be a multiple of 128, at most %d", what, Cout, KL_MAXC);
+    if (Cin % 16 != 0 || Cin > KL_MAXC) return sonet::fail(SONET_ERR_UNSUPPORTED, "%s: Cin=%d must be a multiple of 16, at most %d", what, Cin, KL_MAXC);
+    if (G * GK > 128) return sonet::fail(SONET_ERR_UNSUPPORTED, "%s: G GK = %d columns exceed a block", what, G * GK);
+    const long long Lp = (long long)sonet_knn_stage_columns(B, M, K), Lm = (long long)sonet_node_stage_columns(B, M);
+    const long long nblk = Lp / 128;
+    const int KC = Cin / 16, NS = sonet::ceil_div(KC, KL_STAGE), KCP = NS * KL_STAGE, CT = Cout / 32;
+    if (nblk > 0x7FFFFFFFll || (double)KC * 64.0 * (double)Lm >= 2.0e9 || (double)(Cout / 16) * 64.0 * (double)Lout >= 2.0e9 || (double)CT * KCP * 2048.0 >= 2.0e9)
+        return sonet::fail(SONET_ERR_UNSUPPORTED, "%s: a panel exceeds 2 GiB", what);
+    KnnLayerArgs a;
+    a.rec = reinterpret_cast<const int4 *>(rec); a.zp = reinterpret_cast<const uint4 *>(z_p16); a.wl = wl; a.scale1 = scale1; a.shift1 = shift1;
+    a.Wp = reinterpret_cast<const uint4 *>(Wp); a.scale2 = scale2; a.shift2 = shift2; a.yp = static_cast<char *>(yp); a.rlog = sonet::range_log();
+    a.Lm = Lm; a.relu1 = relu1; a.relu2 = relu2; a.KC = KC; a.NS = NS; a.KCP = KCP; a.CT = CT; a.Cout = Cout; a.GK = GK; a.G = G; a.ngout = ngout; a.Lout = Lout;
+    a.abl = 0;
+#ifdef SONET_VARIANTS
+    sonet::knob_int("SONET_KL_ABL", &a.abl);
+#endif
+    with_int_c<1, 2, 3, 4>(Cout / 128, [&](auto mt) {
+        hipLaunchKernelGGL((knn_layer2_gmax_kernel<decltype(mt)::value>), dim3((unsigned)nblk), dim3(256), 0, sonet::as_stream(stream), a);
+    });
+    return sonet::launched(what);
+}
diff --git a/so-net_amd/csrc/node_stage.hip b/so-net_amd/csrc/node_stage.hip
--- a/so-net_amd/csrc/node_stage.hip
+++ b/so-net_amd/csrc/node_stage.hip
@@ -1,4 +1,5 @@
 #include "common.hpp"
+#include "knn_h1.hpp"
 
 namespace {
 
@@ -81,15 +82,11 @@
         const int grp = (int)blockIdx.y + j * gstride;
         const int c = (grp * KS_CPW + i) * 16 + p16_channel(h, e);
         const bool in = grp < ngrp && c < C;
-        coef[0][t] = in ? 32.f * wl[c * 3 + 0] : 0.f;
-        coef[1][t] = in ? 32.f * wl[c * 3 + 1] : 0.f;
-        coef[2][t] = in ? 32.f * wl[c * 3 + 2] : 0.f;
-        coef[3][t] = in ? scale[c] : 0.f;
-        coef[4][t] = in ? 32.f * shift[c] : 0.f;
-    }
-    const bool valid = r.x != -2, ok = r.x >= 0;
-    const f32x2_t d0 = {__int_as_float(r.y), __int_as_float(r.y)}, d1 = {__int_as_float(r.z), __int_as_float(r.z)},
-                d2 = {__int_as_float(r.w), __int_as_float(r.w)};
+#pragma unroll
+        for (int kind = 0; kind < 5; ++kind) coef[kind][t] = knn_h1_coef(kind, in, c, wl, scale, shift);
+    }
+    const KnnCol kcol = knn_col(r);
+    const bool ok = kcol.ok;
     RangeAcc xr = {0, 0u};
     const float lo = relu ? 0.f : -65504.f;
     const uint4 *zbase = zp + (long long)hh * Lm + (ok ? r.x : 0);
@@ -116,29 +113,15 @@
 #pragma unroll
         for (int i = 0; i < KS_CPW; ++i) {
             if (grp * KS_CPW + i >= KC) break;
-            const unsigned zh[4] = {zhq[i].x, zhq[i].y, zhq[i].z, zhq[i].w}, zm[4] = {zmq[i].x, zmq[i].y, zmq[i].z, zmq[i].w};
-            unsigned hv[4], mv[4];
-#pragma unroll
-            for (int q = 0; q < 4; ++q) {
-                const int slot = (j * KS_CPW + i) * 16 + hh * 8 + 2 * q;
-                const f32x2_t w0 = *reinterpret_cast<const f32x2_t *>(&coef[0][slot]), w1 = *reinterpret_cast<const f32x2_t *>(&coef[1][slot]),
-                            w2 = *reinterpret_cast<const f32x2_t *>(&coef[2][slot]), sc = *reinterpret_cast<const f32x2_t *>(&coef[3][slot]),
-                            sh = *reinterpret_cast<const f32x2_t *>(&coef[4][slot]);
-                const f16x2_t zh2 = __builtin_bit_cast(f16x2_t, zh[q]), zm2 = __builtin_bit_cast(f16x2_t, zm[q]);
-                f32x2_t a = __builtin_convertvector(zh2, f32x2_t) + __builtin_convertvector(zm2, f32x2_t);
-                a = __builtin_elementwise_fma(w0, d0, a);
-                a = __builtin_elementwise_fma(w1, d1, a);
-                a = __builtin_elementwise_fma(w2, d2, a);
-                a = __builtin_elementwise_fma(a, sc, sh);
-                if (!valid) a = f32x2_t{0.f, 0.f};
-                range_track(xr, a[0], a[1]);
-                p16_split2(__builtin_amdgcn_fmed3f(a[0], lo, 65504.f), __builtin_amdgcn_fmed3f(a[1], lo, 65504.f), hv[q], mv[q]);
-            }
+            const int slot = (j * KS_CPW + i) * 16 + hh * 8;
+            const float *const cf[5] = {&coef[0][slot], &coef[1][slot], &coef[2][slot], &coef[3][slot], &coef[4][slot]};
+            uint4 hv, mv;
+            knn_h1_half(zhq[i], zmq[i], cf, kcol, lo, xr, hv, mv);
 #ifdef SONET_VARIANTS
-            if ((abl & 1) && hv[0] != 0x12345u) { hq += 4 * Lp; continue; }
+            if ((abl & 1) && hv.x != 0x12345u) { hq += 4 * Lp; continue; }
 #endif
-            hq[0] = make_uint4(hv[0], hv[1], hv[2], hv[3]);
-            hq[2 * Lp] = make_uint4(mv[0], mv[1], mv[2], mv[3]);
+            hq[0] = hv;
+            hq[2 * Lp] = mv;
             hq += 4 * Lp;
         }
     };
@@ -157,15 +140,7 @@
         }
     }
     if (rlog != nullptr) {
-        unsigned bits;
-        if (relu) {
-            const unsigned pos = xr.mp > 0 ? (unsigned)xr.mp : 0u, nan_neg = xr.mn > 0xFF800000u ? (xr.mn & 0x7FFFFFFFu) : 0u;
-            bits = pos > nan_neg ? pos : nan_neg;
-        } else {
-            bits = range_amax_bits(xr);
-        }
-        unsigned wm = wave_umax(bits);
-        wm = wm > (5u << 23) ? wm - (5u << 23) : 0u;
+        const unsigned wm = range_x32_out(wave_umax(range_act_bits(xr, relu)));
         if ((threadIdx.x & 63) == 0) wmax[threadIdx.x >> 6] = wm;
         __syncthreads();
         if (threadIdx.x == 0) {
diff --git a/so-net_amd/csrc/pointmlp_h3p.hip b/so-net_amd/csrc/pointmlp_h3p.hip
--- a/so-net_amd/csrc/pointmlp_h3p.hip
+++ b/so-net_amd/csrc/pointmlp_h3p.hip
@@ -161,8 +161,6 @@
     __builtin_amdgcn_sched_group_barrier(0x008, NC == 2 ? 3 : 2, 0);
 }
 
-constexpr int GM_STRIDE = 136;
-__device__ __forceinline__ float nan_max(float m, float v) { return (v > m || v != v) ? v : m; }
 __device__ __forceinline__ void lds_barrier() { asm volatile("s_waitcnt lgkmcnt(0)\n\ts_barrier" ::: "memory"); }
 
 template <int MT, int NC, int OCC, int EPI, int OUT>
@@ -353,13 +351,7 @@
                         }
                         const long long n_out = (long long)wg_col * a.G + g;
                         if (n_out < a.ngout) {
-                            range_track(yr, m0, m1);
-                            unsigned hv, mv;
-                            p16_split2(__builtin_amdgcn_fmed3f(m0, split_lo * 32.f, 65504.f), __builtin_amdgcn_fmed3f(m1, split_lo * 32.f, 65504.f), hv, mv);
-                            unsigned *dst = reinterpret_cast<unsigned *>(static_cast<char *>(a.yp)
-                                + ((((size_t)((ct0 + mt) * 2 + qq) * 2) * 2 + h2) * (size_t)a.Lout + (size_t)n_out) * 16) + p;
-                            dst[0] = hv;
-                            dst[(size_t)a.Lout * 8] = mv;
+                            gmax_p16_store(m0, m1, split_lo, yr, a.yp, (ct0 + mt) * 2 + qq, h2, p, (size_t)a.Lout, (size_t)n_out);
                         }
                     }
                 } else {
diff --git a/so-net_amd/models/networks.py b/so-net_amd/models/networks.py
--- a/so-net_amd/models/networks.py
+++ b/so-net_amd/models/networks.py
@@ -225,10 +225,15 @@
         z = _ops.pointmlp_h3p(xp, k1._packed_p16(lambda: k1._weight2d().detach()[:, 3:], "feat"), _ops.const_vec(C1, 1.0, dev),
                               _ops.const_vec(C1, 0.0, dev), False, C1, out="p16", tag="flat")
         s1, t1 = k1._eval_affine()
-        h1 = _ops.knn_stage_input(prep, z, k1._lead_cols(3), s1, t1, k1.activation == 'relu')
+        s2, t2 = k2._eval_affine()
         center, cp = prep["center"], prep["center_p16"]
-        s2, t2 = k2._eval_affine()
-        knn = _ops.pointmlp_h3p_gmax(h1, k2._packed_p16(), s2, t2, k2.activation == 'relu', k2.conv.out_channels, K, G, B * M, out="p16", Lout=xp.L)
+        C2 = k2.conv.out_channels
+        if _ops.KNN_FUSED_LAYER2 and _ops.knn_layer2_supported(C1, C2, K, B, M, xp.L):
+            knn = _ops.knn_layer2_gmax(prep, z, k1._lead_cols(3), s1, t1, k1.activation == 'relu', k2._packed_p16(), s2, t2,
+                                       k2.activation == 'relu', C2, xp.L)
+        else:
+            h1 = _ops.knn_stage_input(prep, z, k1._lead_cols(3), s1, t1, k1.activation == 'relu')
+            knn = _ops.pointmlp_h3p_gmax(h1, k2._packed_p16(), s2, t2, k2.activation == 'relu', C2, K, G, B * M, out="p16", Lout=xp.L)
         s3, t3 = f1._eval_affine()
         h3 = _ops.pointmlp_h3p(knn, f1._packed_p16(lambda: torch.cat((f1._weight2d().detach()[:, 3:], f1._weight2d().detach()[:, :3]), dim=1), "rot3"),
                                s3, t3, f1.activation == 'relu', f1.conv.out_channels, x2=cp, out="p16", tag="flat")
diff --git a/so-net_amd/sonet_hip/_lib.py b/so-net_amd/sonet_hip/_lib.py
--- a/so-net_amd/sonet_hip/_lib.py
+++ b/so-net_amd/sonet_hip/_lib.py
@@ -122,6 +122,7 @@
     "sonet_knn_stage_prepare_f32": [_vp, _vp, _i, _i, _i, _i, _i, _vp, _vp, _vp, _vp],
     "sonet_knn_stage_input_p16": [_vp, _vp, _vp, _vp, _vp, _i, _i, _i, _i, _i, _vp, _vp],
     "sonet_pointmlp_h3p_gmax": [_vp, _i, _vp, _i, _vp, _vp, _vp, _i, _i, _i, _i, _i, _i, _i, _vp, _vp, _vp],
+    "sonet_knn_layer2_gmax_p16": [_vp, _vp, _vp, _vp, _vp, _i, _i, _i, _i, _i, _vp, _vp, _vp, _i, _i, _i, _i, _i, _i, _vp, _vp],
     "sonet_node_stage_columns": [_i, _i],
     "sonet_p16_flat_to_bcm_f32": [_vp, _vp, _i, _i, _i, _vp],
     "sonet_som_sort_group_f32": [_vp, _vp, _vp, _vp, _vp, _i, _i, _i, _i, _vp, _vp, _vp, _vp, _vp, _vp, _vp, _vp],
diff --git a/so-net_amd/sonet_hip/ops.py b/so-net_amd/sonet_hip/ops.py
--- a/so-net_amd/sonet_hip/ops.py
+++ b/so-net_amd/sonet_hip/ops.py
@@ -766,6 +766,7 @@
 NODE_LINEAR_SPLIT = _os.environ.get("SONET_NODE_LINEAR_SPLIT", "1") != "0"
 P16_CHAINS = _os.environ.get("SONET_P16_CHAINS", "1") != "0"
 NODE_STAGE_P16 = _os.environ.get("SONET_NODE_STAGE_P16", "1") != "0"
+KNN_FUSED_LAYER2 = _os.environ.get("SONET_KNN_FUSED_LAYER2", "1") != "0"
 POOLED_TRAIN_EPILOGUE = _os.environ.get("SONET_POOLED_TRAIN_EPILOGUE", "1") != "0"
 H3_SEGPOOL = _os.environ.get("SONET_H3_SEGPOOL", "1") != "0"
 H3_NORM_ON_LOAD = _os.environ.get("SONET_H3_NORM_ON_LOAD", "1") != "0"
@@ -1752,6 +1753,50 @@
         check(_lib.load().sonet_knn_stage_input_p16(ptr(prep["rec"]), ptr(z.data), ptr(wl), ptr(scale), ptr(shift), int(bool(relu)),
                                                     prep["B"], prep["M"], prep["K"], C, ptr(h1.data), stream_ptr()), "sonet_knn_stage_input_p16")
     return h1
+
+
+KNN_LAYER2_MAX_C = 512
+
+
+def knn_layer2_supported(Cin, Cout, K, B=1, M=1, Lout=None):
+    if not (Cout % 128 == 0 and 0 < Cout <= KNN_LAYER2_MAX_C and Cin % 16 == 0 and 0 < Cin <= KNN_LAYER2_MAX_C
+            and 1 <= K <= 128 and min(16, 128 // K) * K <= 128 and B > 0 and M > 0):
+        return False
+    G = min(16, 128 // K)
+    Lm = node_stage_columns(B, M)
+    Lout = Lm if Lout is None else int(Lout)
+    nblk = (B * M + G - 1) // G
+    KCP = (Cin + 127) // 128 * 8
+    return (nblk <= 0x7FFFFFFF and (Cin // 16) * 64.0 * Lm < 2.0e9 and (Cout // 16) * 64.0 * Lout < 2.0e9
+            and (Cout // 32) * KCP * 2048.0 < 2.0e9)
+
+
+def knn_layer2_gmax(prep, z, wl, s1, t1, relu1, wp, s2, t2, relu2, Cout, Lout):
+    if not isinstance(z, P16) or z.B != 1 or z.L != node_stage_columns(prep["B"], prep["M"]):
+        raise SonetHipError("knn_layer2_gmax: z is a P16 1 x C x Lm activation")
+    if wp.dtype != torch.int32:
+        raise SonetHipError("knn_layer2_gmax: an h3p pack (ops.pointmlp_h3p_pack)")
+    _chk(wl, "wl", torch.float32, 2)
+    for n_, v_ in (("s1", s1), ("t1", t1), ("s2", s2), ("t2", t2)):
+        _chk(v_, n_, torch.float32, 1)
+    C = z.C
+    if tuple(wl.shape) != (C, 3) or s1.numel() != C or t1.numel() != C or s2.numel() != Cout or t2.numel() != Cout:
+        raise SonetHipError("knn_layer2_gmax: wl C x 3, s1 / t1 C, s2 / t2 Cout")
+    dev = _same_device(prep["rec"], z.data, wl, s1, t1, wp, s2, t2)
+    lib = _lib.load()
+    if wp.numel() * 4 != lib.sonet_pointmlp_h3p_pack_size(C, Cout):
+        raise SonetHipError("packed weight has %d bytes, expected %d for Cin=%d Cout=%d"
+                            % (wp.numel() * 4, lib.sonet_pointmlp_h3p_pack_size(C, Cout), C, Cout))
+    B, M, K, G = prep["B"], prep["M"], prep["K"], prep["G"]
+    ngout, Lout = B * M, int(Lout)
+    yp = p16_flat(Cout, Lout, ngout, dev)
+    name = "pointmlph3p_knn_gmax%d_%dx%d_L%d" % (K, C, Cout, ngout * K)
+    _range_arm(name)
+    with _lib.on_device(dev), _timed(name):
+        check(lib.sonet_knn_layer2_gmax_p16(ptr(prep["rec"]), ptr(z.data), ptr(wl), ptr(s1), ptr(t1), int(bool(relu1)), B, M, K, C,
+                                            ptr(wp), ptr(s2), ptr(t2), int(bool(relu2)), int(Cout), K, G, ngout, Lout, ptr(yp.data),
+                                            stream_ptr()), "sonet_knn_layer2_gmax_p16")
+    return yp
 
 
 def p16_flat_to_bcm(p, B, M):
```
